# BioinformaticsArchive/HSA

Measured on AMD Instinct MI355X. Metric: aligned reads/sec, 100bp synthetic vs hg19-sized 2BWT, at 1/2/4/8 MI355X, higher is better.
Workload: dtype u32

## Files before the change

### hsa_amd/csrc/hsa_index.hip

```cpp
#include <chrono>
#include <cstring>
#include <hip/hip_runtime.h>
#include <rocprim/rocprim.hpp>
#include <stdarg.h>
#include <stdio.h>
#include <stdlib.h>
#include <string.h>

#include "hsa_device.h"
#include "hsa_internal.h"
#include "hsa_trie.h"

static thread_local char g_err[1024] = "";
int g_waves_per_cu = 16;
int g_pool_entries = 0;
int g_batch_k = getenv("HSA_BATCH_K") ? atoi(getenv("HSA_BATCH_K")) : 32;
int g_batch_idle = getenv("HSA_BATCH_IDLE") ? atoi(getenv("HSA_BATCH_IDLE")) : 768;
int g_hit_cap = 64;

void hsa_set_error(const char *fmt, ...)
{
    va_list ap;
    va_start(ap, fmt);
    vsnprintf(g_err, sizeof g_err, fmt, ap);
    va_end(ap);
}

extern "C" const char *hsa_last_error(void) { return g_err; }
extern "C" void hsa_gpu_set_error_text(const char *msg) { hsa_set_error("%s", msg); }

extern "C" int hsa_device_count(void)
{
    int n = 0;
    if (hipGetDeviceCount(&n) != hipSuccess) return 0;
    return n;
}

extern "C" void hsa_free(void *p) { free(p); }

extern "C" int hsa_configure(int waves_per_cu, int pool_entries, int hit_cap)
{
    if (waves_per_cu > 0) g_waves_per_cu = waves_per_cu;
    if (pool_entries > 0) {
        if (pool_entries > 65535) { hsa_set_error("pool_entries > 65535"); return HSA_E_ARG; }
        g_pool_entries = pool_entries;
    } else if (pool_entries < 0) {
        g_pool_entries = 0;
    }
    if (hit_cap > 0) g_hit_cap = hit_cap;
    return 0;
}

static void hsa_log_alloc(const char *what, size_t bytes, std::chrono::steady_clock::time_point t0)
{
    const double ms = std::chrono::duration<double, std::milli>(std::chrono::steady_clock::now() - t0).count();
    if (ms > 5.0 && getenv("HSA_VERBOSE")) fprintf(stderr, "[hsa] %s: hipMalloc of %.2f GB took %.1f ms\n", what, bytes / 1e9, ms);
}

int hsa_realloc_device(void **out, void **old, size_t bytes)
{
    *out = nullptr;
    if (hipMalloc(out, bytes) != hipSuccess) {
        (void)hipGetLastError();
        *out = nullptr;
        (void)hipFree(*old);
        *old = nullptr;
        if (hipMalloc(out, bytes) != hipSuccess) {
            (void)hipGetLastError();
            *out = nullptr;
            hsa_set_error("hipMalloc(%zu) failed", bytes);
            return HSA_E_MEM;
        }
        return 0;
    }
    (void)hipFree(*old);
    *old = nullptr;
    return 0;
}

int hsa_grow(void **p, size_t *cap, size_t need)
{
    if (need <= *cap && *p) return 0;
    size_t n = need + need / 4 + 4096;
    const auto t0 = std::chrono::steady_clock::now();
    void *np = nullptr;
    *cap = 0;
    if (hsa_realloc_device(&np, p, n)) return HSA_E_MEM;
    *p = np;
    *cap = n;
    hsa_log_alloc("buffer", n, t0);
    return 0;
}

void hsa_scratch_free(SearchScratch &s)
{
    (void)hipFree(s.pool); (void)hipFree(s.nxt); (void)hipFree(s.hbuf);
    const size_t lb = s.link_bytes;
    s = SearchScratch();
    s.link_bytes = lb;
}

extern "C" int hsa_index_release_scratch(hsa_index_t *ix)
{
    if (!ix) { hsa_set_error("hsa_index_release_scratch: null handle"); return HSA_E_ARG; }
    (void)hipSetDevice(ix->device);
    HSA_HIP(hipStreamSynchronize(ix->stream));
    hsa_scratch_free(ix->main); hsa_scratch_free(ix->big); hsa_scratch_free(ix->huge);
    void **bufs[] = {&ix->d_pf, &ix->d_pf2, &ix->d_sp, &ix->d_any, &ix->d_any_aux, &ix->d_help, &ix->d_hp, &ix->d_rf,
                     &ix->d_ch, &ix->d_sm};
    size_t *caps[] = {&ix->d_pf_cap, &ix->d_pf2_cap, &ix->d_sp_cap, &ix->d_any_cap, &ix->d_any_aux_cap, &ix->d_help_cap,
                      &ix->d_hp_cap, &ix->d_rf_cap, &ix->d_ch_cap, &ix->d_sm_cap};
    for (int i = 0; i < 10; ++i) {
        if (*bufs[i]) (void)hipFree(*bufs[i]);
        *bufs[i] = nullptr;
        *caps[i] = 0;
    }
    return 0;
}

int hsa_scratch_reserve(SearchScratch &s, size_t lanes, size_t pcap, size_t hcap, size_t link_bytes)
{
    const size_t pe = lanes * pcap, he = lanes * hcap;
    auto fail = [&]() {
        hsa_set_error("scratch allocation failed (lanes %zu, pool %zu, hits %zu)", lanes, pcap, hcap);
        (void)hipGetLastError();
        hsa_scratch_free(s);
        return HSA_E_MEM;
    };
    if (!s.pool || pe > s.pool_entries || link_bytes != s.link_bytes) {
        const size_t npe = pe > s.pool_entries ? pe : s.pool_entries;
        const auto t0 = std::chrono::steady_clock::now();
        void *np = nullptr, *nn = nullptr;
        if (hsa_realloc_device(&np, (void **)&s.pool, npe * sizeof(uint4)) ||
            hsa_realloc_device(&nn, &s.nxt, npe * link_bytes)) {
            (void)hipFree(np);
            return fail();
        }
        s.pool = (uint4 *)np; s.nxt = nn;
        s.pool_entries = npe;
        s.link_bytes = link_bytes;
        hsa_log_alloc("search scratch pool", npe * (sizeof(uint4) + link_bytes), t0);
    }
    if (!s.hbuf || he > s.hit_entries) {
        const size_t nhe = he > s.hit_entries ? he : s.hit_entries;
        const auto t0 = std::chrono::steady_clock::now();
        void *nh = nullptr;
        if (hsa_realloc_device(&nh, (void **)&s.hbuf, nhe * 9 * sizeof(uint32_t))) return fail();
        s.hbuf = (uint32_t *)nh;
        s.hit_entries = nhe;
        hsa_log_alloc("search scratch hits", nhe * 9 * sizeof(uint32_t), t0);
    }
    return 0;
}

__global__ void k_msb_to_lsb(uint32_t *w, size_t n, uint32_t T)
{
    size_t i = (size_t)blockIdx.x * blockDim.x + threadIdx.x;
    if (i >= n) return;
    uint32_t x = w[i];
    x = (x >> 16) | (x << 16);
    x = ((x & 0xFF00FF00u) >> 8) | ((x & 0x00FF00FFu) << 8);
    x = ((x & 0xF0F0F0F0u) >> 4) | ((x & 0x0F0F0F0Fu) << 4);
    x = ((x & 0xCCCCCCCCu) >> 2) | ((x & 0x33333333u) << 2);
    if (i == n - 1 && (T & 15)) x &= (1u << (2 * (T & 15))) - 1u;
    w[i] = x;
}

// ... 711 lines not shown
```

### hsa_amd/csrc/hsa_search.hip

```cpp
#include "hsa_search_launch.h"
#include "hsa_splice_prefetch.h"

#include <memory>
#include <vector>

#ifdef HSA_DIAG
extern "C" int hsa_diag_read(unsigned long long *out, int n_blocks)
{
    HSA_HIP(hipMemcpyFromSymbol(out, HIP_SYMBOL(g_diag), sizeof(unsigned long long) * 4 * (size_t)n_blocks));
    return 0;
}
extern "C" int hsa_diag_counters(unsigned long long *out, int reset)
{
    HSA_HIP(hipMemcpyFromSymbol(out, HIP_SYMBOL(g_dctr), sizeof(unsigned long long) * 32));
    if (reset) {
        unsigned long long z[32] = {0};
        HSA_HIP(hipMemcpyToSymbol(HIP_SYMBOL(g_dctr), z, sizeof z));
    }
    return 0;
}
#endif

struct MgHost {
    const hsa_mg_job_t *mg;
// ... 112 lines not shown
}

static int export_widths(const HostIn &in, const HostStage &H)
{
    const MgHost *mh = in.mh;
    std::vector<int32_t> cw(2 * mh->width_pairs + 2);
    HSA_HIP(hipMemcpy(cw.data(), H.io.mg.d_cw, mh->width_pairs * 8, hipMemcpyDeviceToHost));
    for (int j = 0; j < in.n; ++j)
        memcpy(mh->widths_out + 2 * mh->mg[j].wb_off, cw.data() + 2 * mh->mg[j].wb_off, 8 * ((size_t)in.jobs[j].len + 1));
    return 0;
}

static void add_stats(hsa_stats_t *stats, const unsigned long long *ctr, float ms, bool main)
{
    if (!stats) return;
    stats->rank_queries += ctr[CTR_RANK]; stats->blocks_loaded += ctr[CTR_SECTORS]; stats->pops += ctr[CTR_POPS];
    stats->kernel_ms += ms;
    if (main) { stats->main_kernel_ms += ms; stats->main_launches += 1; }
}

static long search_any_host(hsa_index_t *ix, const hsa_regime_t *regimes, int n_regimes, const HostIn &in,
                            const HostOut &out)
{
    HSA_HIP(hipSetDevice(ix->device));
    hipStream_t st = ix->stream;
    const hsa_job_t *jobs = in.jobs;
    uint32_t max_len = 1, max_seed = 0;
    for (int j = 0; j < in.n; ++j) {
        if (jobs[j].len > max_len) max_len = jobs[j].len;
        const bool own = in.mh ? in.mh->mg[j].seed == HSA_SEED_OWN : (int)jobs[j].len > jobs[j].seed_len;
        if (own && (uint32_t)jobs[j].seed_len > max_seed) max_seed = (uint32_t)jobs[j].seed_len;
    }
    AnyBufs AB;
    int rc = any_prepare(ix, regimes, n_regimes, (size_t)in.n, st, AB);
    if (rc) return rc;
    HostStage H;
    if ((rc = stage_host(ix, in, nullptr, 0, st, H))) return rc;
    H.io.max_len = (int)max_len; H.io.max_seed = (int)max_seed;
    HSA_HIP(hipMemsetAsync(H.io.ctr, 0, CTR_SLOTS * sizeof(unsigned long long), st));
    HSA_HIP(hipEventRecord(ix->ev0, st));
    if ((rc = any_passes<uint32_t>(ix, AB, H.io, nullptr, st))) return rc;
    HSA_HIP(hipEventRecord(ix->ev1, st));
    unsigned long long ctr[CTR_SLOTS];
    if ((rc = copy_back(H.io, in.n, out, ctr, st))) return rc;
    if (ctr[CTR_ERRORS]) { hsa_set_error("%llu reads pushed a score past the regime's n_stacks", ctr[CTR_ERRORS]); return HSA_E_ARG; }
    if (ctr[CTR_UNFINISHED]) { hsa_set_error("%llu reads exceed the large-pass capacity", ctr[CTR_UNFINISHED]); return HSA_E_ARG; }
    float ms = 0;
    HSA_HIP(hipEventElapsedTime(&ms, ix->ev0, ix->ev1));
    const uint64_t total = ctr[CTR_HITS] < H.io.hit_cap ? ctr[CTR_HITS] : H.io.hit_cap;
    HostHits h = alloc_hits(total);
    if (!h) return HSA_E_MEM;
    if (total) HSA_HIP(hipMemcpy(h.get(), H.io.hits, total * 36, hipMemcpyDeviceToHost));
    if (in.mh && (rc = export_widths(in, H))) return rc;
    add_stats(out.stats, ctr, ms, true);
    *out.hits = h.release();
    return (long)total;
}

static long search_batch_impl(hsa_index_t *ix, const hsa_regime_t *regimes, int n_regimes, const HostIn &in,
                              const HostOut &out);

static long search_split(hsa_index_t *ix, const hsa_regime_t *regimes, int n_regimes, const HostIn &in, const HostOut &out,
                         bool fast_rg)
{
    const MgHost *mh = in.mh;
    hsa_stats_t *stats = out.stats;
    std::vector<int> part[2];
    for (int j = 0; j < in.n; ++j) part[fast_rg && in.jobs[j].len <= FAST_MAX_LEN ? 0 : 1].push_back(j);
    HostHits hs[2] = {HostHits(nullptr, free), HostHits(nullptr, free)};
    long tot[2] = {0, 0};
    if (stats) memset(stats, 0, sizeof *stats);
    for (int k = 0; k < 2; ++k) {
        const int m = (int)part[k].size();
        if (m == 0) continue;
        std::vector<hsa_job_t> pj(m);
        std::vector<hsa_mg_job_t> pm(mh ? m : 0);
        for (int q = 0; q < m; ++q) {
            pj[q] = in.jobs[part[k][q]];
            if (mh) pm[q] = mh->mg[part[k][q]];
        }
        const MgHost pmh = mh ? MgHost{pm.data(), mh->widths, mh->width_pairs, mh->widths_out} : MgHost{};
        std::vector<int32_t> na(m);
        std::vector<uint32_t> fl(m);
        std::vector<uint64_t> ho(m);
        hsa_stats_t ps{};
        uint32_t *ph = nullptr;
        const HostIn pin{pj.data(), m, in.codes, in.codes_len, mh ? &pmh : nullptr};
        const HostOut pout{na.data(), fl.data(), ho.data(), &ph, &ps};
        const long t = k == 0 ? search_batch_impl(ix, regimes, n_regimes, pin, pout)
                              : search_any_host(ix, regimes, n_regimes, pin, pout);
        hs[k].reset(ph);
        if (t < 0) return t;
        tot[k] = t;
        for (int q = 0; q < m; ++q) {
            const int j = part[k][q];
            out.n_aln[j] = na[q]; out.flags[j] = fl[q]; out.hit_off[j] = ho[q] + (k ? (uint64_t)tot[0] : 0);
        }
        if (stats) {
            stats->rank_queries += ps.rank_queries; stats->blocks_loaded += ps.blocks_loaded; stats->pops += ps.pops;
            stats->overflow_reruns += ps.overflow_reruns; stats->kernel_ms += ps.kernel_ms;
            stats->main_kernel_ms += ps.main_kernel_ms; stats->main_launches += ps.main_launches;
        }
    }
    HostHits h = alloc_hits((uint64_t)tot[0] + (uint64_t)tot[1]);
    if (!h) return HSA_E_MEM;
    if (tot[0]) memcpy(h.get(), hs[0].get(), (size_t)tot[0] * 36);
    if (tot[1]) memcpy(h.get() + (size_t)tot[0] * 9, hs[1].get(), (size_t)tot[1] * 36);
    *out.hits = h.release();
    return tot[0] + tot[1];
}

static long search_batch_impl(hsa_index_t *ix, const hsa_regime_t *regimes, int n_regimes, const HostIn &in,
                              const HostOut &out)
{
    const hsa_job_t *jobs = in.jobs;
    const int n_jobs = in.n;
    const size_t codes_len = in.codes_len;
    const MgHost *mh = in.mh;
    hsa_stats_t *stats = out.stats;
    *out.hits = nullptr;
    if (n_regimes < 1 || n_regimes > 2) { hsa_set_error("1 or 2 regimes"); return HSA_E_ARG; }
    if (int rc0 = hsa_need32(ix)) return rc0;
    int rc = check_regimes(regimes, n_regimes);
    if (rc) return rc;
    int max_len, max_seed;
    if ((rc = jobs_limits(jobs, n_jobs, max_len, max_seed))) return rc;
    if (mh && (rc = mg_limits(jobs, mh->mg, n_jobs, *mh, max_seed))) return rc;
    if (codes_len >= 0xFFFFFFFFull) { hsa_set_error("read codes of one call must be < 4 GiB"); return HSA_E_ARG; }
    HSA_HIP(hipSetDevice(ix->device));
    for (int j = 0; j < n_jobs; ++j)
        if (jobs[j].off > codes_len || jobs[j].len > codes_len - jobs[j].off) {
            hsa_set_error("job %d: codes [%llu, +%u) past codes_len %zu", j, (unsigned long long)jobs[j].off,
                          jobs[j].len, codes_len);
            return HSA_E_ARG;
        }
    const bool fast_rg = fast_regimes(regimes, n_regimes);
    bool all_fit = fast_rg;
    for (int j = 0; j < n_jobs && all_fit; ++j) all_fit = jobs[j].len <= FAST_MAX_LEN;
    if (!all_fit) return search_split(ix, regimes, n_regimes, in, out, fast_rg);
    hipStream_t st = ix->stream;
    if (stats) memset(stats, 0, sizeof *stats);
    if (n_jobs == 0) { *out.hits = (uint32_t *)calloc(9, 4); return 0; }
    static const bool verbose = getenv("HSA_VERBOSE") != nullptr;
    const auto now = []() { struct timespec t; clock_gettime(CLOCK_MONOTONIC, &t); return t.tv_sec + 1e-9 * t.tv_nsec; };
    const double tv0 = verbose ? now() : 0.0;

    HostStage H;
    if ((rc = stage_host(ix, in, regimes, n_regimes, st, H))) return rc;
    H.io.max_len = max_len; H.io.max_seed = max_seed;
    LaunchPlan P;
    RegimePlan R = regime_plan(regimes, n_regimes);
    R.nb = H.nb;
    R.nib_ok = R.nib_ok && !mh;
    for (int j = 0; j < n_jobs && R.nib_ok; ++j) R.nib_ok = jobs[j].max_diff <= 6;
    if ((rc = plan_launch(ix, n_jobs, max_len, max_seed, R, PASS_MAIN, P))) return rc;
    HSA_HIP(hipEventRecord(ix->ev0, st));
    if ((rc = launch_pass(ix, P, ix->main, H.io, PassLink{}, st))) return rc;
    HSA_HIP(hipEventRecord(ix->ev1, st));
    unsigned long long ctr[CTR_SLOTS];
    if ((rc = copy_back(H.io, n_jobs, out, ctr, st))) return rc;
    if (ctr[CTR_ERRORS]) { hsa_set_error("%llu reads exceed the regime's max_diff bound", ctr[CTR_ERRORS]); return HSA_E_ARG; }
    float ms = 0;
    HSA_HIP(hipEventElapsedTime(&ms, ix->ev0, ix->ev1));
    uint64_t total = ctr[CTR_HITS] < H.io.hit_cap ? ctr[CTR_HITS] : H.io.hit_cap;
    const double tv1 = verbose ? now() : 0.0;
    HostHits h = alloc_hits(total);
    if (!h) return HSA_E_MEM;
    if (total) HSA_HIP(hipMemcpy(h.get(), H.io.hits, total * 36, hipMemcpyDeviceToHost));
    if (verbose)
        fprintf(stderr, "[hsa] search of %d reads: copies in + kernels + result arrays out %.1f ms (kernels %.1f ms), "
                        "hits out %.1f ms\n", n_jobs, 1e3 * (tv1 - tv0), ms, 1e3 * (now() - tv1));
    add_stats(stats, ctr, ms, true);

    std::vector<int32_t> list, n2;
    std::vector<uint32_t> f2;
    std::vector<uint64_t> o2;
    for (int round = 0; round < 4; ++round) {
        list.clear();
        for (int j = 0; j < n_jobs; ++j) if (out.flags[j] & HSA_F_OVERFLOW) list.push_back(j);
        const int n_over = (int)list.size();
        if (n_over == 0) break;
        n2.resize(n_jobs); f2.resize(n_jobs); o2.resize(n_jobs);
        if (stats) stats->overflow_reruns += n_over;
        LaunchPlan B;
        const int mode = round == 0 ? PASS_BIG : PASS_HUGE;
        if ((rc = plan_launch(ix, n_over, max_len, max_seed, R, mode, B))) return rc;
        const uint64_t cap2 = (uint64_t)n_over * 256 * (round + 1) + 65536;
        const size_t o2_fl = al((size_t)n_jobs * 4), o2_ho = o2_fl * 2, o2_hits = o2_ho + al((size_t)n_jobs * 8);
        DevBuf d2;
        HSA_HIP(hipMalloc(&d2.p, o2_hits + cap2 * 36));
        HSA_HIP(hipMemcpyAsync(H.d_list, list.data(), sizeof(int32_t) * n_over, hipMemcpyHostToDevice, st));
        char *c2 = (char *)d2.p;
        PassIO io2 = H.io;
        io2.list = H.d_list; io2.n = n_over;
        io2.n_aln = (int32_t *)c2; io2.flags = (uint32_t *)(c2 + o2_fl); io2.hit_off = (uint64_t *)(c2 + o2_ho);
        io2.hits = (uint32_t *)(c2 + o2_hits); io2.hit_cap = cap2;
        HSA_HIP(hipEventRecord(ix->ev0, st));
        if ((rc = launch_pass(ix, B, mode == PASS_BIG ? ix->big : ix->huge, io2, PassLink{}, st))) return rc;
        HSA_HIP(hipEventRecord(ix->ev1, st));
        if ((rc = copy_back(io2, n_jobs, HostOut{n2.data(), f2.data(), o2.data(), nullptr, nullptr}, ctr, st))) return rc;
        HSA_HIP(hipEventElapsedTime(&ms, ix->ev0, ix->ev1));
        const uint64_t t2 = ctr[CTR_HITS] < cap2 ? ctr[CTR_HITS] : cap2;
        uint32_t *grown = (uint32_t *)realloc(h.get(), (total + t2 + 1) * 36);
        if (!grown) { hsa_set_error("host allocation of %llu hits failed", (unsigned long long)(total + t2)); return HSA_E_MEM; }
        (void)h.release(); h.reset(grown);
        if (t2) HSA_HIP(hipMemcpy(h.get() + total * 9, io2.hits, t2 * 36, hipMemcpyDeviceToHost));
        for (const int j : list) { out.n_aln[j] = n2[j]; out.flags[j] = f2[j]; out.hit_off[j] = o2[j] + total; }
        total += t2;
        add_stats(stats, ctr, ms, false);
    }
    for (int j = 0; j < n_jobs; ++j)
        if (out.flags[j] & HSA_F_OVERFLOW) { hsa_set_error("read %d exceeds the large-pass capacity", j); return HSA_E_ARG; }
    if (mh && (rc = export_widths(in, H))) return rc;
    *out.hits = h.release();
    return (long)total;
}

extern "C" long hsa_search_batch(hsa_index_t *ix, const hsa_regime_t *regimes, int n_regimes, const hsa_job_t *jobs,
                                 int n_jobs, const uint8_t *codes, size_t codes_len, int32_t *n_aln, uint32_t *flags,
                                 uint64_t *hit_off, uint32_t **hits_out, hsa_stats_t *stats)
{
    return search_batch_impl(ix, regimes, n_regimes, HostIn{jobs, n_jobs, codes, codes_len, nullptr},
                             HostOut{n_aln, flags, hit_off, hits_out, stats});
}

extern "C" long hsa_match_gap_batch(hsa_index_t *ix, const hsa_regime_t *regimes, int n_regimes, const hsa_job_t *jobs,
                                    const hsa_mg_job_t *mg, int n_jobs, const uint8_t *codes, size_t codes_len,
                                    const int32_t *widths, size_t width_pairs, int32_t *widths_out, int32_t *n_aln,
                                    uint64_t *hit_off, uint32_t **hits_out, hsa_stats_t *stats)
{
    *hits_out = nullptr;
    if (n_jobs > 0 && (!mg || !widths || !widths_out)) { hsa_set_error("hsa_match_gap_batch: null argument"); return HSA_E_ARG; }
    std::vector<uint32_t> flags((size_t)(n_jobs > 0 ? n_jobs : 0) + 1);
    const MgHost mh{mg, widths, width_pairs, widths_out};
    return search_batch_impl(ix, regimes, n_regimes, HostIn{jobs, n_jobs, codes, codes_len, &mh},
                             HostOut{n_aln, flags.data(), hit_off, hits_out, stats});
}

extern "C" int hsa_search_device(hsa_index_t *ix, const hsa_regime_t *regimes, int n_regimes,
                                 const hsa_device_batch_t *b, void *stream)
{
    if (int rc = hsa_need32(ix)) return rc;
    return search_device_impl<uint32_t>(ix, regimes, n_regimes, b, stream);
}

extern "C" int hsa_pass_times(hsa_index_t *ix, int n, float *widths_ms, float *search_ms)
{
    if (n < 1 || n > hsa_index::PASS_RING || (uint64_t)n > ix->pev_n) {
        hsa_set_error("hsa_pass_times: %d passes requested, %llu recorded (ring %d)", n,
                      (unsigned long long)ix->pev_n, hsa_index::PASS_RING);
        return HSA_E_ARG;
    }
    for (int i = 0; i < n; ++i) {
        hipEvent_t *pe = ix->pev[(ix->pev_n - (uint64_t)n + (uint64_t)i) % hsa_index::PASS_RING];
        HSA_HIP(hipEventSynchronize(pe[2]));
        HSA_HIP(hipEventElapsedTime(widths_ms + i, pe[0], pe[1]));
        HSA_HIP(hipEventElapsedTime(search_ms + i, pe[1], pe[2]));
    }
    return 0;
}

extern "C" int hsa_last_pass_ms(hsa_index_t *ix, float *widths_ms, float *search_ms)
{
    if (ix->pev_n) return hsa_pass_times(ix, 1, widths_ms, search_ms);
    HSA_HIP(hipEventSynchronize(ix->ev1));
    HSA_HIP(hipEventElapsedTime(widths_ms, ix->ev0, ix->evm));
    HSA_HIP(hipEventElapsedTime(search_ms, ix->evm, ix->ev1));
    return 0;
}
```

### hsa_amd/csrc/hsa_search_kernels.h

```cpp
#pragma once
#include <hip/hip_runtime.h>
#include <stdio.h>
#include <stdlib.h>
#include <string.h>

#include <type_traits>

#include "hsa_device.h"
#include "hsa_internal.h"
#include "hsa_trie.h"

#define NIL16 0xFFFFu
#define BLOCK 256
#define MAXB 128
#define MAXS 512

enum : uint32_t { PH_IDLE = 0, PH_POP, PH_EXACT, PH_EXPAND, PH_EXIT, PH_END, PH_WAIT };

struct SearchArgs {
    RankDir fwd, rev;
    uint32_t T;
    uint32_t C[5];
    RankDir64 fwd64, rev64;
    uint64_t T64;
    uint64_t C64[5];
    const hsa_regime_t *regimes;
    const uint8_t *bmap;
    uint32_t ntab;
    const hsa_job_t *jobs;
    const int32_t *job_list;
    int n_jobs;
    const uint8_t *codes;
    int32_t *n_aln;
    uint32_t *flags;
    uint64_t *hit_off;
    uint32_t *hits;
    uint64_t hit_cap;
    unsigned long long *ctr;
    const uint8_t *wb, *ws;
    uint32_t *wg;
    uint32_t rb, rs, rg;
    uint4 *pool;
    void *nxt;
    uint32_t *hbuf;
    uint32_t pcap, hcap, nb;
    uint32_t off_heads, off_wb, off_ws;
    uint32_t nib_wb, nib_ws;
    uint32_t mm_buckets;
    int32_t *ovf_list;
    const unsigned long long *n_dev;
    uint32_t qctr;
    uint32_t ovf_ctr;
    const hsa_mg_job_t *mg;
    int32_t *cw;
    int32_t *wbid;
    uint32_t *wq;
    uint32_t batch_k;
    uint32_t batch_idle;
    uint32_t split;
    int32_t *sp_n;
    uint64_t *sp_off;
    uint32_t *sp_q, *sp_p;
    const void *ktw;
    uint32_t ktd;
    uint8_t *wkey;
    const int32_t *perm;
    uint32_t okey;
    int32_t *fwd_list;
    unsigned long long *fwd_n;
    uint32_t fwd_only;
    int32_t *rmap;
    uint32_t fr_budget, fr_demand, fr_cap;
    uint32_t *fr_ent;
    uint32_t *fr_tag;
    uint32_t *fr_rq;
    uint32_t *fr_st;
    unsigned long long *fr_q, *fr_p;
    unsigned long long *fr_c;
    const void *stw;
    uint32_t sdc;
};
#define FR_HIT 0x80000000u
#define FR_DONE 0x40000000u
#define FR_EW 8u
#define FR_CH 16u
#define FR_WALK 1024u
#ifndef HSA_HELPERS
#define HSA_HELPERS 1
#endif

typedef const __attribute__((address_space(4))) SearchArgs *ColdArgs;
__device__ __forceinline__ ColdArgs cold_args()
{
    ColdArgs p = (ColdArgs)(__builtin_amdgcn_kernarg_segment_ptr());
    asm volatile("" : "+s"(p));
    return p;
}

__device__ __forceinline__ uint32_t meta_pack(uint32_t i, uint32_t st, uint32_t isd, uint32_t mm, uint32_t go,
                                              uint32_t ge)
{
    return i | st << 10 | isd << 12 | mm << 13 | go << 20 | ge << 24;
}
#define M_I(m) ((int)((m) & 1023u))
#define M_ST(m) ((int)(((m) >> 10) & 3u))
#define M_ISD(m) ((int)(((m) >> 12) & 1u))
#define M_MM(m) ((int)(((m) >> 13) & 127u))
#define M_GO(m) ((int)(((m) >> 20) & 15u))
#define M_GE(m) ((int)((m) >> 24))

#define C_PH(c) ((c) & 7u)
#define C_STRAND(c) (((c) >> 3) & 1u)
#define C_SEED(c) (((c) >> 4) & 1u)
#define C_REG(c) (((c) >> 5) & 1u)
#define C_VT(c) (((c) >> 6) & 1u)
#define C_ALIAS(c) (((c) >> 7) & 1u)
#define C_OVF(c) (((c) >> 8) & 3u)
#define C_LEN(c) ((int)(((c) >> 10) & 1023u))
#define C_SLEN(c) ((int)(((c) >> 20) & 1023u))
#define SET_PH(c, p) ((c) = ((c) & ~7u) | (p))

template <typename V>
__device__ __forceinline__ V pick4(const V v[4], uint32_t c)
{
    return hsa_sel4<V>(c, v[0], v[1], v[2], v[3]);
}

template <typename IT> struct Ix;
template <> struct Ix<uint32_t> {
    __device__ static const RankDir &fwd(const SearchArgs &a) { return a.fwd; }
    __device__ static const RankDir &rev(const SearchArgs &a) { return a.rev; }
    __device__ static uint32_t T(const SearchArgs &a) { return a.T; }
    __device__ static const uint32_t *C(const SearchArgs &a) { return a.C; }
};
template <> struct Ix<uint64_t> {
    __device__ static const RankDir64 &fwd(const SearchArgs &a) { return a.fwd64; }
    __device__ static const RankDir64 &rev(const SearchArgs &a) { return a.rev64; }
    __device__ static uint64_t T(const SearchArgs &a) { return a.T64; }
    __device__ static const uint64_t *C(const SearchArgs &a) { return a.C64; }
};

template <typename IT> struct Ent {
    IT x, y, z;
    uint32_t w;
};
#ifndef HSA_WAVES_SIMD
#define HSA_WAVES_SIMD 4
#endif
#ifndef HSA_POOL_CHUNK
#define HSA_POOL_CHUNK 1
#endif
template <typename IT>
__device__ __forceinline__ size_t pool_base(size_t wv, uint32_t pcap, int lane)
{
#if HSA_POOL_CHUNK
    return (sizeof(IT) == 4 ? 1u : 2u) * wv * (size_t)((pcap + 31u) & ~31u) * 64 + (size_t)lane * 4;
#else
    return (sizeof(IT) == 4 ? 1u : 2u) * wv * pcap * 64 + (size_t)lane;
#endif
}
template <typename IT>
__device__ __forceinline__ size_t ent_at(size_t base, uint32_t slot)
{
#if HSA_POOL_CHUNK
    constexpr uint32_t EQ = sizeof(IT) == 4 ? 4u : 2u, U = sizeof(IT) == 4 ? 1u : 2u;
    return base + (size_t)(slot / EQ) * 256 + (slot % EQ) * U;
#else
    return base + (size_t)slot * (sizeof(IT) == 4 ? 64 : 128);
#endif
}
template <typename IT>
__device__ __forceinline__ Ent<IT> ent_load(const uint4 *pool, size_t base, uint32_t slot)
{
    const size_t i = ent_at<IT>(base, slot);
    if constexpr (sizeof(IT) == 4) {
        const uint4 v = pool[i];
        return Ent<IT>{v.x, v.y, v.z, v.w};
    } else {
        const uint4 u = pool[i], v = pool[i + (HSA_POOL_CHUNK ? 1 : 64)];
        return Ent<IT>{(uint64_t)u.x | (uint64_t)u.y << 32, (uint64_t)u.z | (uint64_t)u.w << 32,
                       (uint64_t)v.x | (uint64_t)v.y << 32, v.z};
    }
}
template <typename IT>
__device__ __forceinline__ void ent_store(uint4 *pool, size_t base, uint32_t slot, const Ent<IT> &e)
{
    const size_t i = ent_at<IT>(base, slot);
    if constexpr (sizeof(IT) == 4) {
        pool[i] = make_uint4(e.x, e.y, e.z, e.w);
    } else {
        pool[i] = make_uint4((uint32_t)e.x, (uint32_t)(e.x >> 32), (uint32_t)e.y, (uint32_t)(e.y >> 32));
        pool[i + (HSA_POOL_CHUNK ? 1 : 64)] = make_uint4((uint32_t)e.z, (uint32_t)(e.z >> 32), e.w, 0u);
    }
}
template <typename IT> struct HitW { static constexpr uint32_t STAGE = sizeof(IT) == 4 ? 9u : 10u;
                                     static constexpr uint32_t OUT = sizeof(IT) == 4 ? 9u : 14u; };

template <int MW> struct BMask;
template <> struct BMask<0> {
    uint32_t m0 = 0;
    __device__ __forceinline__ void clear() { m0 = 0; }
    __device__ __forceinline__ bool any() const { return m0 != 0; }
    __device__ __forceinline__ int lowest() const { return m0 ? __ffs(m0) - 1 : (1 << 30); }
    __device__ __forceinline__ bool test(int b) const { return (m0 >> b) & 1u; }
    __device__ __forceinline__ void set(int b) { m0 |= 1u << b; }
    __device__ __forceinline__ void reset(int b) { m0 &= ~(1u << b); }
};
template <> struct BMask<1> {
    uint64_t m0 = 0;
    __device__ __forceinline__ void clear() { m0 = 0; }
    __device__ __forceinline__ bool any() const { return m0 != 0; }
    __device__ __forceinline__ int lowest() const { return m0 ? __ffsll((unsigned long long)m0) - 1 : (1 << 30); }
    __device__ __forceinline__ bool test(int b) const { return (m0 >> b) & 1ull; }
    __device__ __forceinline__ void set(int b) { m0 |= 1ull << b; }
    __device__ __forceinline__ void reset(int b) { m0 &= ~(1ull << b); }
};
template <> struct BMask<2> {
    uint64_t m0 = 0, m1 = 0;
    __device__ __forceinline__ void clear() { m0 = m1 = 0; }
    __device__ __forceinline__ bool any() const { return (m0 | m1) != 0; }
    __device__ __forceinline__ int lowest() const
    {
        if (m0) return __ffsll((unsigned long long)m0) - 1;
        if (m1) return 64 + __ffsll((unsigned long long)m1) - 1;
        return 1 << 30;
    }
    __device__ __forceinline__ bool test(int b) const { return b < 64 ? ((m0 >> b) & 1ull) : ((m1 >> (b - 64)) & 1ull); }
    __device__ __forceinline__ void set(int b) { if (b < 64) m0 |= 1ull << b; else m1 |= 1ull << (b - 64); }
    __device__ __forceinline__ void reset(int b) { if (b < 64) m0 &= ~(1ull << b); else m1 &= ~(1ull << (b - 64)); }
};

template <typename WT> struct WFmt {
    static constexpr bool NIB = false;
    static constexpr uint32_t BIDB = sizeof(WT) == 1 ? 4u : 8u;
    static constexpr uint32_t BIDM = (1u << BIDB) - 1u;
    static constexpr uint32_t EQ = 1u << BIDB;
    static constexpr uint32_t CSH = BIDB + 1u;
    static constexpr uint32_t EB = 8u * sizeof(WT);
    static constexpr uint32_t EPW = 4u / sizeof(WT);
    __device__ static uint32_t code_bits(uint32_t c) { return (c & 3u) << CSH | (c > 3 ? 4u : 0u) << CSH; }
    __device__ static uint32_t code(uint32_t v) { return (v >> CSH) & 7u; }
};

struct WNib { uint8_t v; };
template <> struct WFmt<WNib> {
    static constexpr bool NIB = true;
    static constexpr uint32_t BIDB = 3u, BIDM = 7u, EQ = 8u, EB = 4u, EPW = 8u;
};

__device__ __forceinline__ uint32_t nib4(uint32_t x)
{
    uint32_t b = x & 0x0F0F0F0Fu;
    const uint32_t ge7 = ((b + 0x09090909u) >> 4) & 0x01010101u;
    b = (b & ~(ge7 * 0x0Fu)) | ge7 * 7u;
    uint32_t n = b | ((x >> 4) & 0x01010101u) << 3;
    n = (n | n >> 4) & 0x00FF00FFu;
    return (n | n >> 8) & 0xFFFFu;
}

#ifdef HSA_DIAG
static __device__ unsigned long long g_diag[8192 * 4];
static __device__ unsigned long long g_dctr[32];
#define DC(i) (++dc[i])
#else
#define DC(i) ((void)0)
#endif

template <typename IT> struct WChain {
    IT k, l;
    uint32_t bid;
    IT prevw;
    uint32_t acc;
    uint32_t tl, tix;
    uint32_t lr;
};

template <typename WT, typename IT>
__device__ __forceinline__ void width_step(const SearchArgs &a, WChain<IT> &ch, uint32_t t, uint32_t n, uint32_t c,
                                           uint32_t cbits, uint32_t *__restrict__ brow, IT *__restrict__ wrow,
                                           uint32_t &st_q, uint32_t &st_b, uint32_t &st_t)
{
    using F = WFmt<WT>;
    IT w;
    if (t < n) {
        if (c < 4) {
            if (ch.tl < a.ktd) {
                ch.tix = ch.tix * 4u + c;
                ++ch.tl;
                trie_w_load<IT>(a.ktw, trie_base(ch.tl) + ch.tix, ch.k, ch.l);
                ++st_t;
            } else {
                IT ok, ol;
                st_b += occ1_pair(Ix<IT>::rev(a), ch.k, ch.l + 1u, c, ok, ol);
                const IT cc = pick4(Ix<IT>::C(a), c);
                ch.k = cc + ok + 1u;
                ch.l = cc + ol;
            }
            st_q += 2;
        }
        if (ch.k > ch.l || c > 3) { ch.k = 0; ch.l = Ix<IT>::T(a); ++ch.bid; ch.tl = 0; ch.tix = 0; ch.lr = t; }
        w = ch.l - ch.k + 1u;
    } else {
        w = 0; ++ch.bid;
    }
    if (t > 0) {
        if (ch.prevw == w) ch.acc |= F::EQ << (((t - 1) % F::EPW) * F::EB);
        if ((t - 1) % F::EPW == F::EPW - 1) { brow[((t - 1) / F::EPW) * 64] = ch.acc; ch.acc = 0; }
    }
    ch.acc |= ((ch.bid < F::BIDM ? ch.bid : F::BIDM) | cbits) << ((t % F::EPW) * F::EB);
    if (wrow) wrow[t * 64] = w;
    ch.prevw = w;
    if (t == n) brow[(t / F::EPW) * 64] = ch.acc;
}

struct WRow { uint32_t q, b, t, bid, tail; };

__device__ __forceinline__ uint8_t cost_key(const SearchArgs &a, const WRow &w)
{
    const uint32_t b = w.bid < 15u ? w.bid : 15u;
    if (!a.okey) return (uint8_t)(w.bid < 255u ? w.bid : 255u);
    return (uint8_t)(b << 4 | (w.tail < 16u ? 2u : w.tail < 48u ? 1u : 0u));
}

template <typename WT, typename IT>
__device__ __forceinline__ WRow width_row(const SearchArgs &a, uint32_t R, uint32_t strand, const hsa_job_t &J)
{
    using F = WFmt<WT>;
    const uint32_t len = J.len;
    const uint64_t off = J.off;
    const bool has_seed = (int)len > J.seed_len;
    const uint32_t slen = has_seed ? (uint32_t)J.seed_len : 0u;
    const size_t rb = R >> 6, rl = R & 63u;
    uint32_t *const brow = reinterpret_cast<uint32_t *>(const_cast<uint8_t *>(a.wb)) + rb * (a.rb / 4) * 64 + rl;
    uint32_t *const srow = reinterpret_cast<uint32_t *>(const_cast<uint8_t *>(a.ws)) + rb * (a.rs / 4) * 64 + rl;
    IT *const wrow = reinterpret_cast<IT *>(a.wg) + rb * a.rg * 64 + rl;
    WChain<IT> f{0, Ix<IT>::T(a), 0, 0, 0, 0, 0}, sd{0, Ix<IT>::T(a), 0, 0, 0, 0, 0};
    uint32_t st_q = 0, st_b = 0, st_t = 0;
    const uint32_t s0 = len - slen;
#ifndef HSA_CODECACHE
#define HSA_CODECACHE 1
#endif
    uint32_t cq[2] = {0xFFFFFFFFu, 0xFFFFFFFFu}, cword[2] = {0u, 0u};
    auto base = [&](uint32_t sp, int ch) -> uint32_t {
        const uint64_t ix = off + (strand ? len - 1u - sp : sp);
        uint32_t c;
        if constexpr (HSA_CODECACHE) {
            const uint32_t wq = (uint32_t)(ix >> 2);
            if (wq != cq[ch]) {
                cword[ch] = *reinterpret_cast<const uint32_t *>(a.codes + (ix & ~(uint64_t)3));
                cq[ch] = wq;
            }
            c = (cword[ch] >> (((uint32_t)ix & 3u) * 8u)) & 0xFFu;
        } else {
            c = a.codes[ix];
        }
        return strand && c < 4 ? 3u - c : c;
    };
    for (uint32_t t = 0; t <= len; ++t) {
        const uint32_t cf = t < len ? base(t, 0) : 4u;
        width_step<WT, IT>(a, f, t, len, cf, t < len ? F::code_bits(cf) : 0u, brow, wrow, st_q, st_b, st_t);
        if (has_seed && t <= slen) {
            const uint32_t cs = t < slen ? base(s0 + t, 1) : 4u;
            width_step<WT, IT>(a, sd, t, slen, cs, 0u, srow, nullptr, st_q, st_b, st_t);
        }
    }
    return WRow{st_q, st_b, st_t, f.bid, len - f.lr};
}

__device__ __forceinline__ void wave_add(unsigned long long *c, unsigned long long v)
{
    for (int d = 32; d >= 1; d >>= 1) v += __shfl_xor(v, d);
    if ((threadIdx.x & 63) == 0 && v) atomicAdd(c, v);
}

#define HSA_NOFWD 0xFFFFFFFFu
#define HSA_F_NEEDFWD 0x100u

template <typename WT, typename IT = uint32_t>
__global__ void __launch_bounds__(BLOCK) k_widths(SearchArgs a)
{
    const uint32_t R = blockIdx.x * BLOCK + threadIdx.x;
    const uint32_t n_jobs = a.n_dev ? (uint32_t)*a.n_dev : (uint32_t)a.n_jobs;
    const uint32_t q = R >> 1, strand = R & 1u;
    WRow w{0, 0, 0, 0};
    if (R < 2u * n_jobs) {
        const hsa_job_t J = a.jobs[a.job_list ? a.job_list[q] : (int)q];
        w = width_row<WT, IT>(a, R, strand, J);
        if (!strand) a.wq[q] = w.q;
        if (a.wkey) a.wkey[R] = cost_key(a, w);
    }
    wave_add(&a.ctr[CTR_RANK], strand ? w.q : 0u);
    wave_add(&a.ctr[CTR_WIDTH_Q], strand ? w.q : 0u);
    wave_add(&a.ctr[CTR_FWD_Q_ALL], strand ? 0u : w.q);
    wave_add(&a.ctr[CTR_SECTORS], w.b);
    wave_add(&a.ctr[CTR_TRIE], w.t);
}

template <typename WT, typename IT = uint32_t>
__global__ void __launch_bounds__(BLOCK) k_widths_reads(SearchArgs a, uint32_t mode, int32_t *list2,
                                                        unsigned long long *n2)
{
    const uint32_t p = blockIdx.x * BLOCK + threadIdx.x;
    const uint32_t n_jobs = mode == 3 ? (uint32_t)*n2 : a.n_dev ? (uint32_t)*a.n_dev : (uint32_t)a.n_jobs;
    WRow w{0, 0, 0, 0};
    bool more = false;
    if (p < n_jobs) {
        const uint32_t q = mode == 3 ? (uint32_t)list2[p] : p;
        const hsa_job_t J = a.jobs[a.job_list ? a.job_list[q] : (int)q];
        const uint32_t R = mode == 1 ? q : mode == 3 ? (uint32_t)(((uint32_t)a.n_jobs + 63u) & ~63u) + p : 2u * q;
        w = width_row<WT, IT>(a, R, mode == 1 ? 1u : 0u, J);
        if (mode == 3) a.rmap[q] = (int32_t)R;
        const uint8_t key = cost_key(a, w);
        if (mode == 1) {
            more = (int)w.bid - 1 > J.max_diff;
            a.wq[q] = HSA_NOFWD;
            if (a.wkey) { a.wkey[2 * q + 1] = key; a.wkey[2 * q] = 255u; }
        } else if (mode == 3) {
            a.wq[q] = w.q;
            if (a.wkey) a.wkey[2 * q] = key;
        }
    }
    if (mode == 1) {
        const uint64_t m = __ballot(more);
        const int lane = (int)(threadIdx.x & 63);
        unsigned long long b = 0;
        if (m && lane == __ffsll((unsigned long long)m) - 1) b = atomicAdd(n2, (unsigned long long)__popcll(m));
        b = __shfl(b, __ffsll((unsigned long long)(m ? m : 1ull)) - 1);
        if (more) list2[b + __popcll(m & ((1ull << lane) - 1ull))] = (int32_t)p;
    }
    const uint32_t rq = mode == 1 ? w.q : 0u, fq = mode == 2 ? w.q : 0u, sq = mode == 3 ? w.q : 0u;
    wave_add(&a.ctr[CTR_RANK], rq + fq);
    wave_add(&a.ctr[CTR_WIDTH_Q], rq + fq);
    wave_add(&a.ctr[CTR_FWD_Q_ALL], fq + sq);
    wave_add(&a.ctr[CTR_FWD_Q_REF], fq);
    wave_add(&a.ctr[CTR_SECTORS], w.b);
    wave_add(&a.ctr[CTR_TRIE], w.t);
}

template <typename WT>
__global__ void __launch_bounds__(BLOCK) k_widths_import(SearchArgs a)
{
    using F = WFmt<WT>;
    const uint32_t q = blockIdx.x * BLOCK + threadIdx.x;
    const uint32_t n_jobs = a.n_dev ? (uint32_t)*a.n_dev : (uint32_t)a.n_jobs;
    if (q >= n_jobs) return;
    const int job = a.job_list ? a.job_list[q] : (int)q;
    const hsa_job_t J = a.jobs[job];
    const hsa_mg_job_t M = a.mg[job];
    const uint32_t R = q * 2u + (uint32_t)(M.strand & 1);
    const size_t rb = R >> 6, rl = R & 63u;
    uint32_t *const brow = reinterpret_cast<uint32_t *>(const_cast<uint8_t *>(a.wb)) + rb * (a.rb / 4) * 64 + rl;
    uint32_t *const srow = reinterpret_cast<uint32_t *>(const_cast<uint8_t *>(a.ws)) + rb * (a.rs / 4) * 64 + rl;
    uint32_t *const wrow = a.wg + rb * a.rg * 64 + rl;
    int32_t *const drow = a.wbid + rb * a.rg * 64 + rl;
    const bool prefix = M.seed == HSA_SEED_ALIAS && M.ws_off == HSA_MG_PREFIX;
    auto emit = [&](uint32_t *row, const int32_t *w, uint32_t n, bool read_row) {
        uint32_t acc = 0;
        uint32_t wt = (uint32_t)w[0];
        for (uint32_t t = 0; t <= n; ++t) {
            const uint32_t bid = prefix && t == n ? (n ? (uint32_t)w[2 * t - 1] + 1u : 1u) : (uint32_t)w[2 * t + 1];
            const uint32_t wn = t + 1 < n || (t + 1 == n && !prefix) ? (uint32_t)w[2 * t + 2] : 0u;
            uint32_t e = bid < F::BIDM ? bid : F::BIDM;
            if (t < n && wt == wn) e |= F::EQ;
            if (read_row && t < n) e |= F::code_bits(a.codes[J.off + t]);
            acc |= e << ((t % F::EPW) * F::EB);
            if (t % F::EPW == F::EPW - 1 || t == n) { row[(t / F::EPW) * 64] = acc; acc = 0; }
            if (read_row) { wrow[t * 64] = wt; drow[t * 64] = (int32_t)bid; }
            wt = wn;
        }
    };
    emit(brow, a.cw + 2 * M.wb_off, J.len, true);
    if (M.seed == HSA_SEED_OWN) emit(srow, a.cw + 2 * M.ws_off, (uint32_t)J.seed_len, false);
}

static __global__ void __launch_bounds__(BLOCK) k_widths_export(SearchArgs a)
{
    const uint32_t q = blockIdx.x * BLOCK + threadIdx.x;
    const uint32_t n_jobs = a.n_dev ? (uint32_t)*a.n_dev : (uint32_t)a.n_jobs;
    if (q >= n_jobs) return;
    const int job = a.job_list ? a.job_list[q] : (int)q;
    if (a.flags[job] & HSA_F_OVERFLOW) return;
    const hsa_job_t J = a.jobs[job];
    const hsa_mg_job_t M = a.mg[job];
    if (M.seed == HSA_SEED_ALIAS && M.ws_off == HSA_MG_PREFIX) return;
    const uint32_t R = q * 2u + (uint32_t)(M.strand & 1);
    const size_t base = (R >> 6) * (size_t)a.rg * 64 + (R & 63u);
    int32_t *const o = a.cw + 2 * M.wb_off;
    for (uint32_t t = 0; t <= J.len; ++t) {
        o[2 * t] = (int32_t)a.wg[base + t * 64];
        o[2 * t + 1] = a.wbid[base + t * 64];
    }
}


__device__ __forceinline__ uint32_t order_bin(const SearchArgs &a, uint32_t q)
{
    const uint32_t k0 = a.wkey[2 * q], k1 = a.wkey[2 * q + 1];
    const uint32_t k = k0 < k1 ? k0 : k1;
    if (a.okey) {
        const uint32_t v = (k >> 4) * 3u + (k & 15u);
        return 15u - (v < 15u ? v : 15u);
    }
    return 15u - (k < 15u ? k : 15u);
}

static __global__ void __launch_bounds__(BLOCK) k_order_hist(SearchArgs a, uint32_t *hist)
{
    __shared__ uint32_t h[16];
    if (threadIdx.x < 16) h[threadIdx.x] = 0;
    __syncthreads();
    const uint32_t q = blockIdx.x * BLOCK + threadIdx.x;
    if (q < (uint32_t)a.n_jobs) atomicAdd(&h[order_bin(a, q)], 1u);
    __syncthreads();
    if (threadIdx.x < 16 && h[threadIdx.x]) atomicAdd(&hist[threadIdx.x], h[threadIdx.x]);
}

static __global__ void k_order_scan(uint32_t *hist)
{
    uint32_t s = 0;
    for (int b = 0; b < 16; ++b) { hist[16 + b] = s; s += hist[b]; }
}

static __global__ void __launch_bounds__(BLOCK) k_order_scatter(SearchArgs a, uint32_t *hist, int32_t *perm)
{
    __shared__ uint32_t h[16], base[16];
    if (threadIdx.x < 16) h[threadIdx.x] = 0;
    __syncthreads();
    const uint32_t q = blockIdx.x * BLOCK + threadIdx.x;
    uint32_t b = 0, r = 0;
    if (q < (uint32_t)a.n_jobs) { b = order_bin(a, q); r = atomicAdd(&h[b], 1u); }
    __syncthreads();
    if (threadIdx.x < 16 && h[threadIdx.x]) base[threadIdx.x] = atomicAdd(&hist[16 + threadIdx.x], h[threadIdx.x]);
    __syncthreads();
    if (q < (uint32_t)a.n_jobs) perm[base[b] + r] = (int32_t)q;
}

static __global__ void __launch_bounds__(BLOCK) k_split_finalize(SearchArgs a)
{
    const uint32_t q = blockIdx.x * BLOCK + threadIdx.x;
    const uint32_t n_jobs = a.n_dev ? (uint32_t)*a.n_dev : (uint32_t)a.n_jobs;
    unsigned long long q_add = 0, p_add = 0, w_add = 0;
    if (q < n_jobs) {
        const int job = a.job_list ? a.job_list[q] : (int)q;
        const int32_t nr = a.sp_n[2 * q], nf = a.sp_n[2 * q + 1];
        int32_t na = 0;
        uint32_t fl = 0;
        uint64_t off = 0;
        if (nr < 0 || (nr == 0 && nf < 0)) {
            fl = HSA_F_OVERFLOW;
            if (a.ovf_list) a.ovf_list[atomicAdd(&a.ctr[a.ovf_ctr], 1ull)] = job;
            else atomicAdd(&a.ctr[CTR_UNFINISHED], 1ull);
        } else if (nr > 0) {
            na = nr; off = a.sp_off[2 * q];
            q_add = a.sp_q[2 * q]; p_add = a.sp_p[2 * q];
        } else {
            w_add = a.wq[q];
            q_add = (unsigned long long)a.sp_q[2 * q] + a.sp_q[2 * q + 1] + w_add;
            p_add = (unsigned long long)a.sp_p[2 * q] + a.sp_p[2 * q + 1];
            if (nf > 0) { na = nf; off = a.sp_off[2 * q + 1]; }
            else fl = HSA_F_FALLBACK;
        }
        a.n_aln[job] = na;
        a.flags[job] = fl;
        a.hit_off[job] = off;
    }
    for (int d = 32; d >= 1; d >>= 1) {
        q_add += __shfl_xor(q_add, d);
        p_add += __shfl_xor(p_add, d);
        w_add += __shfl_xor(w_add, d);
    }
    if ((threadIdx.x & 63) == 0) {
        if (q_add) atomicAdd(&a.ctr[CTR_RANK], q_add);
        if (p_add) atomicAdd(&a.ctr[CTR_POPS], p_add);
        if (w_add) { atomicAdd(&a.ctr[CTR_WIDTH_Q], w_add); atomicAdd(&a.ctr[CTR_FWD_Q_REF], w_add); }
    }
}

template <int MW, bool GAPS, typename WT, int NT, bool HUGE = false, typename IT = uint32_t>
__global__ void __launch_bounds__(NT, HSA_WAVES_SIMD) k_search(SearchArgs a)
{
    using F = WFmt<WT>;
    using E = Ent<IT>;
    using CT = typename std::conditional<sizeof(IT) == 8, int64_t, int>::type;
    constexpr uint32_t HW = HitW<IT>::STAGE, OW = HitW<IT>::OUT;
    const IT TT = Ix<IT>::T(a);
    const IT *const CC = Ix<IT>::C(a);
    using LT = typename std::conditional<HUGE, uint32_t, uint16_t>::type;
    constexpr bool FRH = !HUGE && HSA_HELPERS && GAPS && sizeof(IT) == 4 && !WFmt<WT>::NIB;
    constexpr uint32_t NIL = HUGE ? 0xFFFFFFFFu : (uint32_t)NIL16;
    constexpr bool IMP = !GAPS && !HUGE && sizeof(IT) == 4 && !WFmt<WT>::NIB;
#ifdef HSA_DIAG
    if (threadIdx.x == 0 && blockIdx.x < 8192) {
        g_diag[blockIdx.x * 4 + 0] = __builtin_amdgcn_s_memtime();
        g_diag[blockIdx.x * 4 + 1] = __builtin_amdgcn_s_memrealtime();
    }
#endif
    extern __shared__ __align__(16) uint8_t s_lds[];
    const uint32_t tid = threadIdx.x;
    const uint32_t gid = blockIdx.x * NT + tid;
    const int lane = (int)(tid & 63);
    for (uint32_t t = tid; t < 2 * a.ntab; t += NT) s_lds[t] = a.bmap[(t / a.ntab) * MAXS + t % a.ntab];
    static_assert(2 * sizeof(hsa_regime_t) <= 128, "regime LDS slot");
    hsa_regime_t *const s_reg = reinterpret_cast<hsa_regime_t *>(s_lds + 2 * a.ntab);
    if (tid < 2 * sizeof(hsa_regime_t) / 4)
        reinterpret_cast<uint32_t *>(s_reg)[tid] = reinterpret_cast<const uint32_t *>(a.regimes)[tid];
    __syncthreads();
    LT *const s_heads = reinterpret_cast<LT *>(s_lds + a.off_heads);
    using WTL = typename std::conditional<F::NIB, uint8_t, WT>::type;
    WTL *const s_wb = reinterpret_cast<WTL *>(s_lds + a.off_wb);
    WTL *const s_ws = reinterpret_cast<WTL *>(s_lds + a.off_ws);
    uint32_t *const s_nb = reinterpret_cast<uint32_t *>(s_lds + a.off_wb);
    uint32_t *const s_ns = reinterpret_cast<uint32_t *>(s_lds + a.off_ws);
    const size_t wv = gid >> 6;
#if HSA_POOL_CHUNK
    const size_t link0 = wv * (size_t)((a.pcap + 31u) & ~31u) * 64 + (size_t)lane * 32;
#define NXT(s) reinterpret_cast<LT *>(a.nxt)[link0 + (size_t)((s) >> 5) * 2048 + ((s) & 31u)]
#else
    const size_t link0 = wv * a.pcap * 64 + (size_t)lane;
#define NXT(s) reinterpret_cast<LT *>(a.nxt)[link0 + (size_t)(s) * 64]
#endif
    const size_t pbase = pool_base<IT>(wv, a.pcap, lane);
#define HB(i) r->hbuf[(wv * r->hcap * HW + (uint32_t)(i)) * 64 + lane]
#define HEAD(b) s_heads[(uint32_t)(b) * NT + tid]
#define WB(p) s_wb[(((uint32_t)(p) / F::EPW) * NT + tid) * F::EPW + (uint32_t)(p) % F::EPW]
#define WS(p) s_ws[(((uint32_t)(p) / F::EPW) * NT + tid) * F::EPW + (uint32_t)(p) % F::EPW]
#define RG(f) (s_reg[C_REG(ctl)].f)

    uint32_t ctl = PH_IDLE;
    uint32_t qpos = 0;
    uint32_t pen = 0;
    uint32_t rmode = 0;
    uint32_t pos = 0;
    IT ik = 0, il = 0;
    IT aux = 0;
    int opt_max_diff = 0, max_diff = 0, best_score = 0, n_aln = 0, n_entries = 0;
    CT best_cnt = 0;
    uint32_t pool_top = 0;
    uint32_t free_head = NIL;
    uint32_t idle_acc = 0;
    BMask<MW> mask;
    E e{0, 0, 0, 0};
    uint32_t st_p = 0, st_wq = 0, st_q = 0, st_b = 0;
    uint32_t sq0 = 0, sp0 = 0;
    uint32_t frs = 0, fr_p0 = 0, fr_q0 = 0;
    uint32_t fr_tick = 0;
    uint32_t st_hs = 0, st_hq = 0;
    const uint32_t n_jobs = a.n_dev ? (uint32_t)*a.n_dev : (uint32_t)a.n_jobs;
#ifdef HSA_DIAG
    uint32_t dc[21] = {0};
    uint64_t tsec[4] = {0, 0, 0, 0};
    uint64_t tt = 0;
    uint64_t rd_t0 = 0;
    uint32_t rd_steps = 0, rd_p0 = 0;
#define TMARK(k) do { const uint64_t t_ = __builtin_amdgcn_s_memtime(); tsec[k] += t_ - tt; tt = t_; } while (0)
#endif

#define S_MM ((int)(pen & 1023u))
#define S_GO ((int)((pen >> 10) & 1023u))
#define S_GE ((int)(pen >> 20))
#define R_MODE ((int)(rmode & 255u))
#define R_MAXGO ((int)((rmode >> 8) & 255u))
#define R_MAXGE ((int)(rmode >> 16))
#define SCORE(mm, go, ge) ((mm) * S_MM + (go) * S_GO + (ge) * S_GE)

    auto wbg = [&](int p) -> uint32_t {
        if constexpr (F::NIB) return (s_nb[((uint32_t)p >> 3) * NT + tid] >> (((uint32_t)p & 7u) * 4u)) & 15u;
        else return WB(p);
    };
    auto wsg = [&](int p) -> uint32_t {
        if constexpr (F::NIB) return (s_ns[((uint32_t)p >> 3) * NT + tid] >> (((uint32_t)p & 7u) * 4u)) & 15u;
        else return WS(p);
    };
    auto wbs = [&](int p, uint32_t v) {
        if constexpr (F::NIB) {
            uint32_t &w = s_nb[((uint32_t)p >> 3) * NT + tid];
            const uint32_t sh = ((uint32_t)p & 7u) * 4u;
            w = (w & ~(15u << sh)) | v << sh;
        } else {
            WB(p) = (WTL)v;
        }
    };
    const uint8_t *rowp = nullptr;
    uint32_t cur_c = 0;
#ifndef HSA_ROWCACHE
#define HSA_ROWCACHE 1
#endif
    uint32_t rw_q = 0xFFFFFFFFu, rw_w = 0;
    auto getc = [&](int p) -> uint32_t {
        if constexpr (F::NIB && !HSA_ROWCACHE) {
            return WFmt<uint8_t>::code(rowp[((uint32_t)p >> 2) * 256u + ((uint32_t)p & 3u)]);
        } else if constexpr (F::NIB) {
            const uint32_t q = (uint32_t)p >> 2;
            if (q != rw_q) {
                rw_w = *reinterpret_cast<const uint32_t *>(rowp + q * 256u);
                rw_q = q;
            }
            return WFmt<uint8_t>::code((rw_w >> (((uint32_t)p & 3u) * 8u)) & 0xFFu);
        } else {
            return F::code(WB(p));
        }
    };
    auto bucket_of = [&](uint32_t m) -> int {
        if (!GAPS && a.mm_buckets) return M_MM(m);
        const int sc = SCORE(M_MM(m), M_GO(m), M_GE(m));
        return (uint32_t)sc < a.ntab ? (int)s_lds[C_REG(ctl) * a.ntab + sc] : 0xFF;
    };
    auto flush = [&](const E &v, int b) {
        if ((uint32_t)b >= a.nb) { ctl |= 1u << 8; return; }
        uint32_t slot;
        if (HUGE && free_head != NIL) {
            slot = free_head;
            free_head = NXT(slot);
        } else {
            if (pool_top >= a.pcap) { ctl |= 1u << 8; return; }
            slot = pool_top++;
        }
        DC(8);
        ent_store<IT>(a.pool, pbase, slot, v);
        const uint32_t old = mask.test(b) ? (uint32_t)HEAD(b) : NIL;
        NXT(slot) = (LT)old;
        HEAD(b) = (LT)slot;
        mask.set(b);
    };
    auto start_search = [&]() {
        best_score = SCORE(opt_max_diff + 1, R_MAXGO + 1, R_MAXGE + 1);
        max_diff = opt_max_diff;
        best_cnt = 0; n_aln = 0;
        mask.clear(); pool_top = 0; free_head = NIL;
        e = E{0, TT, 0, meta_pack((uint32_t)C_LEN(ctl), ST_M, 0, 0, 0, 0)};
        ctl |= 1u << 6;
        n_entries = 1;
        frs = 0; fr_p0 = st_p;
        SET_PH(ctl, PH_POP);
    };
    auto fr_key = [&]() -> uint32_t { return qpos * 2u + (1u - C_STRAND(ctl)); };
    auto row_base = [&](uint32_t cap_words) -> size_t {
        const int32_t *const rm = cold_args()->rmap;
        const uint32_t r = rm ? (C_STRAND(ctl) ? qpos : (uint32_t)rm[qpos]) : qpos * 2u + C_STRAND(ctl);
        return (size_t)(r >> 6) * cap_words * 64 + (r & 63u);
    };
    auto start_strand = [&]() {
        const ColdArgs r = cold_args();
        const uint32_t *src = reinterpret_cast<const uint32_t *>(r->wb) + row_base(r->rb / 4);
        const uint32_t nwb = r->rb / 4;
        if constexpr (F::NIB) {
            rowp = reinterpret_cast<const uint8_t *>(src);
            rw_q = 0xFFFFFFFFu;
            auto pack = [&](const uint32_t *row, uint32_t nw, uint32_t *dst, uint32_t cap) {
                const uint32_t nn = (nw + 1u) / 2u < cap ? (nw + 1u) / 2u : cap;
                for (uint32_t j = 0; j < nn; j += 4) {
                    uint32_t w[8];
#pragma unroll
                    for (uint32_t u = 0; u < 8; ++u) w[u] = 2u * j + u < nw ? row[(2u * j + u) * 64u] : 0u;
#pragma unroll
                    for (uint32_t u = 0; u < 4; ++u)
                        if (j + u < nn) dst[(j + u) * NT + tid] = nib4(w[2u * u]) | nib4(w[2u * u + 1u]) << 16;
                }
            };
            pack(src, nwb, s_nb, r->nib_wb);
            if (C_SEED(ctl) && !C_ALIAS(ctl))
                pack(reinterpret_cast<const uint32_t *>(r->ws) + row_base(r->rs / 4), r->rs / 4, s_ns, r->nib_ws);
        } else {
        uint32_t *const db = reinterpret_cast<uint32_t *>(s_wb) + (tid & ~63u);
        for (uint32_t q = 0; q < nwb; ++q)
            __builtin_amdgcn_global_load_lds(src + q * 64, db + q * NT, 4, 0, 0);
        if (C_SEED(ctl) && !C_ALIAS(ctl)) {
            const uint32_t *ss = reinterpret_cast<const uint32_t *>(r->ws) + row_base(r->rs / 4);
            uint32_t *const ds = reinterpret_cast<uint32_t *>(s_ws) + (tid & ~63u);
            const uint32_t nws = r->rs / 4;
            for (uint32_t q = 0; q < nws; ++q)
                __builtin_amdgcn_global_load_lds(ss + q * 64, ds + q * NT, 4, 0, 0);
        }
        }
        __builtin_amdgcn_s_waitcnt(0);
        DC(15);
        start_search();
    };
    auto finish_job = [&](uint32_t fl, int na, uint64_t ho) {
        const ColdArgs r = cold_args();
#ifdef HSA_DIAG
        atomicMax(&g_dctr[21], (unsigned long long)rd_steps);
        atomicMax(&g_dctr[22], (unsigned long long)(__builtin_amdgcn_s_memrealtime() - rd_t0));
        atomicMax(&g_dctr[23], (unsigned long long)(st_p - rd_p0));
        atomicMax(&g_dctr[na > 0 ? 24 : 25], (unsigned long long)rd_steps);
#endif
        if (r->split) {
            const uint32_t pi = qpos * 2u + (1u - C_STRAND(ctl));
            r->sp_n[pi] = (fl & HSA_F_OVERFLOW) ? -1 : na;
            r->sp_off[pi] = ho;
            r->sp_q[pi] = st_q - sq0;
            r->sp_p[pi] = st_p - sp0;
            st_q = sq0; st_p = sp0;
            if constexpr (FRH) {
                if (a.fr_budget) {
                    if (frs & 1u) atomicOr(&r->fr_st[pi], FR_DONE);
                    atomicAdd(&r->fr_c[2], 1ull);
                    frs = 0;
                }
            }
            SET_PH(ctl, PH_IDLE);
            return;
        }
        const int job = r->job_list ? r->job_list[qpos] : (int)qpos;
        if (fl & HSA_F_NEEDFWD) {
            r->fwd_list[atomicAdd(r->fwd_n, 1ull)] = job;
            SET_PH(ctl, PH_IDLE);
            return;
        }
        if (fl & HSA_F_OVERFLOW) {
            if (r->ovf_list) r->ovf_list[atomicAdd(&r->ctr[r->ovf_ctr], 1ull)] = job;
            else atomicAdd(&r->ctr[CTR_UNFINISHED], 1ull);
        }
        r->n_aln[job] = na;
        r->flags[job] = fl;
        r->hit_off[job] = ho;
        SET_PH(ctl, PH_IDLE);
    };
    auto help_done = [&]() {
        const ColdArgs r = cold_args();
        const uint32_t key = fr_key();
        const unsigned long long dq = st_q - fr_q0, dp = st_p - fr_p0;
        st_q = fr_q0; st_p = fr_p0;
        const unsigned long long o1 = atomicAdd(&r->fr_q[key], dq), o2 = atomicAdd(&r->fr_p[key], dp);
        asm volatile("s_waitcnt vmcnt(0)" :: "v"(o1), "v"(o2) : "memory");
        atomicSub(&r->fr_st[key], 1u);
        ++st_hs; st_hq += (uint32_t)dq;
        frs = 0;
        SET_PH(ctl, PH_IDLE);
    };
    auto end_strand = [&]() {
        if constexpr (FRH) {
            if (frs & 2u) { help_done(); return; }
        }
        if (n_aln > 0) {
            const ColdArgs r = cold_args();
            const unsigned long long o = atomicAdd(&r->ctr[CTR_HITS], (unsigned long long)n_aln);
            if (o + (uint64_t)n_aln > r->hit_cap) { finish_job(HSA_F_OVERFLOW, 0, 0); return; }
            uint32_t *dst = r->hits + o * OW;
            const uint32_t s30 = C_STRAND(ctl) << 30;
            for (int h = 0; h < n_aln; ++h) {
                const uint32_t end = h == 0 && !r->mg ? (uint32_t)(C_LEN(ctl) - 1) : 0u;
                if constexpr (sizeof(IT) == 4) {
                    const uint32_t v0 = HB(h * 9 + 0), v1 = HB(h * 9 + 1), v2 = HB(h * 9 + 2), v3 = HB(h * 9 + 3),
                                   v4 = HB(h * 9 + 4), v8 = HB(h * 9 + 8);
                    dst[h * 9 + 0] = v0;
                    dst[h * 9 + 1] = v1;
                    dst[h * 9 + 2] = v2;
                    dst[h * 9 + 3] = v3;
                    dst[h * 9 + 4] = v4;
                    dst[h * 9 + 5] = s30;
                    dst[h * 9 + 6] = 0;
                    dst[h * 9 + 7] = end;
                    dst[h * 9 + 8] = v8;
                } else {
                    uint32_t v[10];
#pragma unroll
                    for (int j = 0; j < 10; ++j) v[j] = HB(h * 10 + j);
                    dst[h * 14 + 0] = v[0];
                    dst[h * 14 + 1] = s30;
#pragma unroll
                    for (int j = 1; j < 9; ++j) dst[h * 14 + 1 + j] = v[j];
                    dst[h * 14 + 10] = 0;
                    dst[h * 14 + 11] = end;
                    dst[h * 14 + 12] = v[9];
                    dst[h * 14 + 13] = 0;
                }
            }
            finish_job(0, n_aln, o);
        } else if (cold_args()->mg || cold_args()->split) {
            finish_job(0, 0, 0);
        } else if (C_STRAND(ctl)) {
            const uint32_t wq = cold_args()->wq[qpos];
            if (wq == HSA_NOFWD) {
                finish_job(HSA_F_NEEDFWD, 0, 0);
            } else {
                ctl &= ~(1u << 3);
                st_wq += wq;
                start_strand();
            }
        } else {
            finish_job(HSA_F_FALLBACK, 0, 0);
        }
    };
    auto on_hit = [&](IT k, IT l, IT rk, IT rl) -> bool {
        const ColdArgs r = cold_args();
        if constexpr (FRH) {
            if (frs & 3u) {
                atomicOr(&r->fr_st[fr_key()], FR_HIT);
                if (frs & 2u) return false;
            }
        }
        const uint32_t m = e.w;
        const int score = SCORE(M_MM(m), M_GO(m), M_GE(m));
        if (n_aln == 0) {
            best_score = score;
            const int best_diff = M_MM(m) + M_GO(m) + ((R_MODE & MODE_GAPE) ? M_GE(m) : 0);
            if (!(R_MODE & MODE_NONSTOP)) max_diff = (best_diff + 1 > opt_max_diff) ? opt_max_diff : best_diff + 1;
        }
        if (score == best_score) {
            if constexpr (sizeof(IT) == 4) best_cnt = (int)((uint32_t)best_cnt + (l - k + 1u));
            else best_cnt += (CT)(l - k + 1u);
        } else if (best_cnt > RG(max_top2)) {
            return false;
        }
        bool add = true;
        if (M_GO(m)) {
            for (int j = 0; j < n_aln; ++j) {
                if constexpr (sizeof(IT) == 4) {
                    if (HB(j * 9 + 1) == k && HB(j * 9 + 2) == l) { add = false; break; }
                } else {
                    const uint64_t hk = (uint64_t)HB(j * 10 + 1) | (uint64_t)HB(j * 10 + 2) << 32;
                    const uint64_t hl = (uint64_t)HB(j * 10 + 3) | (uint64_t)HB(j * 10 + 4) << 32;
                    if (hk == k && hl == l) { add = false; break; }
                }
            }
        }
        if (add) {
            if ((uint32_t)n_aln >= r->hcap) { ctl |= 1u << 8; return false; }
            const IT x = l - k + 1u;
            const int ldp = M_ISD(m) ? M_I(m) : 0;
            if (ldp > 0) {
#ifdef HSA_DIAG
// ... 308 lines not shown
                    const uint64_t em = __ballot(elig);
                    if (elig && lane == __ffsll((unsigned long long)em) - 1) {
                        const unsigned long long wt = __hip_atomic_load(&r->fr_c[3], __ATOMIC_RELAXED, __HIP_MEMORY_SCOPE_AGENT);
                        const unsigned long long rs = __hip_atomic_load(&r->fr_c[0], __ATOMIC_RELAXED, __HIP_MEMORY_SCOPE_AGENT);
                        const unsigned long long tk = __hip_atomic_load(&r->fr_c[1], __ATOMIC_RELAXED, __HIP_MEMORY_SCOPE_AGENT);
                        if (wt > rs - tk + a.fr_demand) {
                            if (!fr_offer()) frs |= 4u;
                            else if (frs & 2u) stop = true;
                            else { frs |= 1u; fr_p0 = st_p; fr_q0 = st_q; }
                        }
                    }
                    if (stop) { SET_PH(ctl, PH_END); continue; }
                }
            }
            if (C_VT(ctl)) {
                DC(3);
                ctl &= ~(1u << 6);
            } else {
                DC(4);
                const int b = mask.lowest();
                const uint32_t slot = HEAD(b);
                e = ent_load<IT>(a.pool, pbase, slot);
                const uint32_t nx = NXT(slot);
                if (nx == NIL) mask.reset(b);
                else HEAD(b) = (LT)nx;
                if (HUGE) { NXT(slot) = (LT)free_head; free_head = slot; }
            }
            --n_entries;
            ++st_p;
            const uint32_t m = e.w;
            if (!(R_MODE & MODE_NONSTOP) && SCORE(M_MM(m), M_GO(m), M_GE(m)) > best_score + S_MM) {
                SET_PH(ctl, PH_END);
                continue;
            }
            const int em = m_of(m);
            if (em < 0) { DC(18); continue; }
            const int ei = M_I(m);
            if (ei > 0 && em < (int)(wbg(ei - 1) & F::BIDM)) { DC(18); continue; }
            if (ei == 0) {
                DC(20);
                if (!on_hit(e.x, e.y, e.z, e.z + (e.y - e.x)) && !C_OVF(ctl)) SET_PH(ctl, PH_END);
                continue;
            }
            if (em == 0 && (M_ST(m) == ST_M || (R_MODE & MODE_GAPE) || M_GE(m) == R_MAXGE)) {
                ik = e.x; il = e.y; aux = e.z + (e.y - e.x); pos = (uint32_t)(ei - 1);
                SET_PH(ctl, PH_EXACT);
                continue;
            }
            req = 1; rp1 = e.x; rp2 = e.y + 1u;
            if constexpr (IMP) {
                const uint32_t len = (uint32_t)C_LEN(ctl), dp = len - (uint32_t)ei;
                if (len > a.sdc && dp < a.sdc) req = dp + 1u == a.sdc ? 2 : 4;
            }
            if constexpr (F::NIB) cur_c = getc(ei - 1);
            SET_PH(ctl, PH_EXPAND);
        } while (0);

#ifdef HSA_DIAG
        TMARK(1);
#endif
        IT oa[4], ob[4], srk[4];
#ifdef HSA_DIAG
        {
            const uint64_t rq = __ballot(req == 1);
            if (lane == 0) dc[6] += (uint32_t)__popcll(rq);
            const uint32_t ph0 = C_PH(ctl);
            if (req == 1) DC(ph0 == PH_EXACT ? 1 : 2);
            if (req == 1 && rp2 == rp1 + 1u) DC(ph0 == PH_EXACT ? 16 : 17);
        }
#endif
        uint32_t two = 0;
#ifdef HSA_DIAG
        rd_steps += req == 1 ? 1u : 0u;
#endif
        if constexpr (IMP) {
            if (req == 2) {
                trie_s_load4(a.stw, rp1, oa, ob, srk);
            } else if (req == 3) {
                trie_s_load1(a.stw, rp1, oa[0], ob[0], srk[0]);
            }
        }
        if (req == 1) {
            two = occ_pair(Ix<IT>::fwd(a), rp1, rp2, oa, ob) - 1u;
            st_q += 2u; st_b += 1u + two;
        }

#ifdef HSA_DIAG
        asm volatile("s_waitcnt vmcnt(0)" ::: "memory");
        TMARK(2);
#endif
        const uint32_t ph = C_PH(ctl);
        if (IMP && req == 3) {
            ik = oa[0]; il = ob[0]; aux = srk[0] + (il - ik);
            if (M_I(e.w) != C_LEN(ctl)) e.x = e.y = e.z = 1u;
            --pos;
        } else if (F::NIB && req == 1 && ph == PH_EXACT && cur_c > 3) {
            st_q -= 2u; st_b -= 1u + two;
            SET_PH(ctl, PH_POP);
        } else if (req && ph == PH_EXACT) {
            const uint32_t c = F::NIB ? cur_c : getc((int)pos);
            IT oc = 0;
#pragma unroll
            for (uint32_t d = 1; d < 4; ++d) oc += d > c ? ob[d] - oa[d] : (IT)0;
            const IT cc = pick4(CC, c);
            ik = cc + pick4(oa, c) + 1u;
            il = cc + pick4(ob, c);
            aux -= oc;
            if (ik > il) {
                SET_PH(ctl, PH_POP);
            } else if (pos-- == 0) {
                const IT rk = aux - (il - ik), erl = e.z + (e.y - e.x);
                const IT hk = e.x ? ik : (IT)0, hl = e.y ? il : (IT)0, hrk = e.z ? rk : (IT)0, hrl = erl ? aux : (IT)0;
                SET_PH(ctl, PH_POP);
                if (!on_hit(hk, hl, hrk, hrl) && !C_OVF(ctl)) SET_PH(ctl, PH_END);
            }
        } else if (req && ph == PH_EXPAND) {
            const uint32_t m = e.w;
            const IT ek = e.x, el = e.y, erk = e.z, erl = erk + (el - ek);
            const int i = M_I(m) - 1;
            const int est = M_ST(m), emm = M_MM(m), ego = M_GO(m), ege = M_GE(m);
            const int em = m_of(m);
            const int len = C_LEN(ctl);
            uint32_t ne = 0;
            if (IMP && req != 1) {
                if (req == 4) {
#pragma unroll
                    for (int c = 0; c < 4; ++c) { oa[c] = ek * 4u + (IT)c; ob[c] = 0; srk[c] = 0; }
                }
                ne = 0xFu;
                st_q += 2u;
            } else {
                IT oc = 0;
#pragma unroll
                for (int c = 3; c >= 0; --c) {
                    const IT d = ob[c] - oa[c];
                    oa[c] = CC[c] + oa[c] + 1u;
                    ob[c] = CC[c] + ob[c];
                    srk[c] = (erl - oc) - (ob[c] - oa[c]);
                    oc += d;
                }
#pragma unroll
                for (int c = 0; c < 4; ++c) ne |= (oa[c] <= ob[c] ? 1u : 0u) << c;
            }
            int allow_diff = 1, allow_M = 1;
            if (i > 0) {
                const uint32_t w1 = wbg(i - 1), w0 = wbg(i);
                const int b1 = (int)(w1 & F::BIDM), b0 = (int)(w0 & F::BIDM);
                if (b1 > em - 1) allow_diff = 0;
                else if (b1 == em - 1 && b0 == em - 1 && (w1 & F::EQ)) allow_M = 0;
                const int ii = i - (len - C_SLEN(ctl));
                if (C_SEED(ctl) && ii > 0) {
                    int ems = RG(max_seed_diff) - (emm + ego);
                    if (R_MODE & MODE_GAPE) ems -= ege;
                    const uint32_t s1 = C_ALIAS(ctl) ? wbg(ii - 1) : wsg(ii - 1);
                    const uint32_t s0 = C_ALIAS(ctl) ? wbg(ii) : wsg(ii);
                    const int c1 = (int)(s1 & F::BIDM), c0 = (int)(s0 & F::BIDM);
                    if (c1 > ems - 1) allow_diff = 0;
                    else if (c1 == ems - 1 && c0 == ems - 1 && (s1 & F::EQ)) allow_M = 0;
                }
            }
            const uint32_t sc = F::NIB ? cur_c : getc(i);
            uint32_t cand = 0;
            if constexpr (GAPS) {
                const int ies = RG(indel_end_skip);
                const int tmp = (R_MODE & MODE_LOGGAP) ? hsa_log2((uint32_t)(ege + ego)) / 2 + 1 : ego + ege;
                const bool ok = (allow_diff != 0) & ((R_MAXGO > 0) | (ego > 0)) & (i >= ies + tmp) & (len - i >= ies + tmp);
                const IT occ = el - ek + 1u;
                const uint32_t c_m = ego < R_MAXGO ? (1u | ne << 1) : 0u;
                const uint32_t c_i = ege < R_MAXGE ? 1u : 0u;
                const bool d_ok = (ege < R_MAXGE) & ((ege + ego < max_diff) | (occ < (IT)RG(max_del_occ)));
                const uint32_t c_d = d_ok ? ne << 1 : 0u;
                const uint32_t c_g = est == ST_M ? c_m : est == ST_I ? c_i : c_d;
                cand = ok ? c_g : 0u;
            }
            {
                uint32_t c_mm = 0;
#pragma unroll
                for (int j = 1; j <= 4; ++j) {
                    const uint32_t c = (sc + (uint32_t)j) & 3u;
                    c_mm |= ((ne >> c) & 1u) << (4 + j);
                }
                const uint32_t c_eq = sc < 4 ? ((ne >> (sc & 3u)) & 1u) << 8 : 0u;
                cand |= (allow_diff & allow_M) ? c_mm : c_eq;
            }
            auto entry = [&](uint32_t b) -> E {
                const bool ins = GAPS && b == 0, del = GAPS && b >= 1 && b <= 4;
                const uint32_t c = del ? b - 1u : (sc + b - 4u) & 3u;
                const uint32_t is_mm = (b != 8u || sc > 3) ? 1u : 0u;
                IT k = pick4(oa, c), l = pick4(ob, c), rk = pick4(srk, c);
                uint32_t meta;
                if (GAPS && (ins || del)) {
                    if (ins) { k = ek; l = el; rk = erk; }
                    const uint32_t go = (uint32_t)ego + (est == ST_M), ge = (uint32_t)ege + (est != ST_M);
                    meta = meta_pack((uint32_t)(del ? i + 1 : i), ins ? ST_I : ST_D, 1u, (uint32_t)emm, go, ge);
                } else {
                    meta = meta_pack((uint32_t)i, ST_M, is_mm, (uint32_t)emm + is_mm, (uint32_t)ego, (uint32_t)ege);
                }
                return E{k, l, rk, meta};
            };
#ifdef HSA_DIAG
            auto doomed = [&](uint32_t mw) {
                const int em2 = m_of(mw), i2 = M_I(mw);
                return em2 < 0 || (i2 > 0 && em2 < (int)(wbg(i2 - 1) & F::BIDM));
            };
#endif
            if (cand) {
                const uint32_t last = 31u - (uint32_t)__clz(cand);
                n_entries += __popc(cand);
                uint32_t rest = cand & ~(1u << last);
                if constexpr (HUGE) {
                    for (; rest; rest &= rest - 1u) {
                        const E v = entry((uint32_t)__ffs(rest) - 1u);
#ifdef HSA_DIAG
                        if (doomed(v.w)) DC(19);
#endif
                        flush(v, bucket_of(v.w));
                    }
                } else if (rest) {
                    const uint32_t g_go = (uint32_t)ego + (est == ST_M), g_ge = (uint32_t)ege + (est != ST_M);
                    const uint32_t mI = meta_pack((uint32_t)i, ST_I, 1u, (uint32_t)emm, g_go, g_ge);
                    const uint32_t mD = meta_pack((uint32_t)(i + 1), ST_D, 1u, (uint32_t)emm, g_go, g_ge);
                    const uint32_t mM = meta_pack((uint32_t)i, ST_M, 1u, (uint32_t)emm + 1u, (uint32_t)ego, (uint32_t)ege);
                    const uint32_t mP = meta_pack((uint32_t)i, ST_M, 0u, (uint32_t)emm, (uint32_t)ego, (uint32_t)ege);
                    const int bG = GAPS ? bucket_of(mI) : -1, bM = bucket_of(mM), bP = bucket_of(mP);
                    auto head0 = [&](int b) -> uint32_t {
                        return b >= 0 && (uint32_t)b < a.nb && mask.test(b) ? (uint32_t)HEAD(b) : NIL;
                    };
                    const uint32_t hG0 = GAPS ? head0(bG) : NIL, hM0 = head0(bM), hP0 = head0(bP);
                    uint32_t hG = hG0, hM = hM0, hP = hP0;
                    for (; rest; rest &= rest - 1u) {
                        const uint32_t b = (uint32_t)__ffs(rest) - 1u;
                        const bool ins = GAPS && b == 0, gap = GAPS && b <= 4u;
                        const bool mt = b == 8u && sc < 4;
                        const uint32_t c = gap ? b - 1u : (sc + b - 4u) & 3u;
                        IT k = pick4(oa, c), l = pick4(ob, c), rk = pick4(srk, c);
                        if (ins) { k = ek; l = el; rk = erk; }
                        const uint32_t meta = ins ? mI : gap ? mD : mt ? mP : mM;
                        const int bk = gap ? bG : mt ? bP : bM;
#ifdef HSA_DIAG
                        if (doomed(meta)) DC(19);
#endif
                        if ((uint32_t)bk >= a.nb || pool_top >= a.pcap) { ctl |= 1u << 8; continue; }
                        const uint32_t slot = pool_top++;
                        DC(8);
                        ent_store<IT>(a.pool, pbase, slot, E{k, l, rk, meta});
                        NXT(slot) = (LT)(bk == bG ? hG : bk == bM ? hM : hP);
                        hG = bk == bG ? slot : hG;
                        hM = bk == bM ? slot : hM;
                        hP = bk == bP ? slot : hP;
                    }
                    if (GAPS && hG != hG0) { HEAD(bG) = (LT)hG; mask.set(bG); }
                    if (hM != hM0) { HEAD(bM) = (LT)hM; mask.set(bM); }
                    if (hP != hP0) { HEAD(bP) = (LT)hP; mask.set(bP); }
                }
                const E v = entry(last);
#ifdef HSA_DIAG
                if (doomed(v.w)) DC(19);
#endif
                const int bk = bucket_of(v.w);
                if (bk <= mask.lowest()) { e = v; ctl |= 1u << 6; }
                else flush(v, bk);
            }
            SET_PH(ctl, PH_POP);
        }
#ifdef HSA_DIAG
        TMARK(3);
#endif
    }

#ifdef HSA_DIAG
    __syncthreads();
    if (threadIdx.x == 0 && blockIdx.x < 8192) {
        g_diag[blockIdx.x * 4 + 2] = __builtin_amdgcn_s_memtime();
        g_diag[blockIdx.x * 4 + 3] = __builtin_amdgcn_s_memrealtime();
    }
    for (int i = 0; i < 18; ++i)
        if (i < 9 || i > 12) atomicAdd(&g_dctr[i], (unsigned long long)dc[i]);
    for (int i = 18; i < 21; ++i) atomicAdd(&g_dctr[i], (unsigned long long)dc[i]);
    if (lane == 0)
        for (int i = 0; i < 4; ++i) atomicAdd(&g_dctr[9 + i], (unsigned long long)tsec[i]);
#endif
    if constexpr (FRH) {
        if (a.fr_budget) {
            unsigned long long hs = st_hs, hq = st_hq;
            for (int d = 32; d >= 1; d >>= 1) { hs += __shfl_xor(hs, d); hq += __shfl_xor(hq, d); }
            if (lane == 0) { atomicAdd(&a.fr_c[6], hs); atomicAdd(&a.fr_c[8], hq); }
        }
    }
    atomicAdd(&a.ctr[CTR_RANK], (unsigned long long)st_q);
    atomicAdd(&a.ctr[CTR_SECTORS], (unsigned long long)st_b);
    atomicAdd(&a.ctr[CTR_POPS], (unsigned long long)st_p);
    if (st_wq) {
        atomicAdd(&a.ctr[CTR_RANK], (unsigned long long)st_wq);
        atomicAdd(&a.ctr[CTR_WIDTH_Q], (unsigned long long)st_wq);
        atomicAdd(&a.ctr[CTR_FWD_Q_REF], (unsigned long long)st_wq);
    }
#undef HEAD
#undef WB
#undef WS
#undef NXT
#undef HB
#undef RG
#undef S_MM
#undef S_GO
#undef S_GE
#undef R_MODE
#undef R_MAXGO
#undef R_MAXGE
#undef SCORE
}

// ... 11 lines not shown
```

### hsa_amd/csrc/hsa_search_launch.h

```cpp
#pragma once
#include "hsa_search_kernels.h"

static int check_regimes(const hsa_regime_t *rg, int n)
{
    for (int r = 0; r < n; ++r) {
        const hsa_regime_t &R = rg[r];
        if (R.s_mm < 0 || R.s_gapo < 0 || R.s_gape < 0) { hsa_set_error("negative penalty"); return HSA_E_ARG; }
        if (R.n_stacks <= 0 || R.n_stacks > ANY_MAX_STACKS) {
            hsa_set_error("n_stacks %d outside 1..%d", R.n_stacks, ANY_MAX_STACKS);
            return HSA_E_ARG;
        }
        if (R.max_gapo < 0 || R.max_gape < 0) { hsa_set_error("max_gapo/max_gape negative"); return HSA_E_ARG; }
        if (R.max_diff < -1) { hsa_set_error("max_diff out of range"); return HSA_E_ARG; }
    }
    return 0;
}

static int bucket_map(const hsa_regime_t &R, uint8_t map[MAXS])
{
    bool used[MAXS] = {false};
    const int md = R.max_diff < 0 ? 0 : R.max_diff;
    const int go_max = R.max_gapo < md ? R.max_gapo : md;
    for (int mm = 0; mm <= md + 1; ++mm)
        for (int go = 0; go <= go_max; ++go)
            for (int ge = 0; ge <= (go > 0 ? R.max_gape : 0); ++ge) {
                const int s = mm * R.s_mm + go * R.s_gapo + ge * R.s_gape;
                if (s >= 0 && s < MAXS && s < R.n_stacks) used[s] = true;
            }
    int k = 0;
    for (int s = 0; s < MAXS; ++s) map[s] = used[s] && k < 0xFF ? (uint8_t)k++ : (uint8_t)0xFF;
    return k;
}

static bool fast_regimes(const hsa_regime_t *rg, int n)
{
    if (getenv("HSA_FORCE_ANY")) return false;
    for (int r = 0; r < n; ++r) {
        const hsa_regime_t &R = rg[r];
        if (R.max_gapo > 14 || R.max_gape > 254 || R.max_diff > 125 || R.max_seed_diff > 254 || R.n_stacks > MAXS)
            return false;
        uint8_t map[MAXS];
        if (bucket_map(R, map) > MAXB) return false;
    }
    return true;
}

#define FAST_MAX_LEN 1023u

static bool mm_buckets(const hsa_regime_t *rg, int n, const uint8_t *bmap)
{
    for (int r = 0; r < n; ++r) {
        const hsa_regime_t &R = rg[r];
        if (R.max_gapo != 0 || R.s_mm <= 0) return false;
        const int md = R.max_diff < 0 ? 0 : R.max_diff;
        for (int mm = 0; mm <= md + 1; ++mm) {
            const int sc = mm * R.s_mm;
            if (sc >= MAXS || bmap[r * MAXS + sc] != mm) return false;
        }
    }
    return true;
}

struct RegimePlan {
    int nb;
    bool gaps, wide, nib_ok;
    int max_entries;
};

static RegimePlan regime_plan(const hsa_regime_t *rg, int n)
{
    RegimePlan C{.nb = 0, .gaps = false, .wide = false, .nib_ok = true, .max_entries = 0};
    for (int r = 0; r < n; ++r) {
        const int bound = rg[r].max_diff > rg[r].max_seed_diff ? rg[r].max_diff : rg[r].max_seed_diff;
        C.gaps |= rg[r].max_gapo > 0;
        C.wide |= bound > 14;
        C.nib_ok &= bound <= 6;
        C.max_entries = rg[r].max_entries > C.max_entries ? rg[r].max_entries : C.max_entries;
    }
    return C;
}

struct LaunchPlan {
    size_t lanes, blocks;
    uint32_t nt;
    uint32_t pcap, hcap, nb;
    bool gaps, wide;
    bool nib;
    uint32_t off_heads, off_wb, off_ws;
    uint32_t nib_wb, nib_ws;
    size_t lds;
    bool huge;
    uint32_t ntab;
    size_t resident;
    size_t res_lanes = 0;
};

enum { PASS_MAIN = 0, PASS_BIG = 1, PASS_HUGE = 2 };

static int plan_launch(hsa_index *ix, int n_jobs, int max_len, int max_seed, const RegimePlan &R, int mode,
                       LaunchPlan &P, uint32_t ent_bytes = 16)
{
    const int nb = R.nb, max_entries = R.max_entries;
    const bool gaps = R.gaps, wide = R.wide, nib_ok = R.nib_ok;
    const bool big = mode == PASS_BIG;
    P.huge = mode == PASS_HUGE;
    P.ntab = (uint32_t)ix->staged_ntab;
    P.nb = (uint32_t)nb;
    P.gaps = gaps;
    P.wide = wide;
    const uint32_t esz = wide ? 2u : 1u;
    P.nib = false;
    auto layout = [&](uint32_t nt) {
        const uint32_t epw = P.nib ? 8u : 4u / esz;
        P.nt = nt;
        P.off_heads = 2 * P.ntab + 128;
        P.off_wb = P.off_heads + (uint32_t)nb * nt * (P.huge ? 4u : 2u);
        P.nib_wb = ((uint32_t)max_len + 7u) / 8u;
        P.nib_ws = ((uint32_t)max_seed + 7u) / 8u;
        const uint32_t wbw = P.nib ? P.nib_wb : (uint32_t)max_len / epw + 1u;
        const uint32_t wsw = P.nib ? P.nib_ws : (uint32_t)max_seed / epw + 1u;
        P.off_ws = P.off_wb + wbw * nt * 4u;
        P.lds = ((size_t)P.off_ws + (size_t)wsw * nt * 4u + 15) / 16 * 16;
        int per_cu = (int)((160u * 1024u) / P.lds);
        const int cap = 4 * HSA_WAVES_SIMD / (int)(nt / 64);
        const int want = g_waves_per_cu / (int)(nt / 64);
        if (per_cu > cap) per_cu = cap;
        if (per_cu > want) per_cu = want > 0 ? want : 1;
        return per_cu;
    };
    static const int force256 = getenv("HSA_WG256") != nullptr;
    auto best = [&]() {
        int per_cu = layout(P.huge ? 64 : 256);
        if (per_cu < 4 && !force256 && !P.huge) {
            const int p64 = layout(64);
            if (p64 > per_cu * 4) per_cu = p64;
            else per_cu = layout(256);
        }
        return per_cu;
    };
    int per_cu = best();
    const char *wf = getenv("HSA_WFMT");
    const bool force_nib = wf && !strcmp(wf, "nib"), no_nib = wf && !strcmp(wf, "byte");
    if (nib_ok && !wide && !P.huge && !no_nib && (force_nib || (!gaps && per_cu * (int)(P.nt / 64) < 16))) {
        const int waves8 = per_cu * (int)(P.nt / 64);
        const LaunchPlan keep = P;
        P.nib = true;
        const int per_nib = best();
        if (!force_nib && per_nib * (int)(P.nt / 64) <= waves8) { P = keep; }
        else per_cu = per_nib;
    }
    if (P.lds > 160 * 1024) { hsa_set_error("reads too long for the LDS budget (%zu bytes)", P.lds); return HSA_E_ARG; }
    if (per_cu < 1) { hsa_set_error("search kernel does not fit (LDS %zu)", P.lds); return HSA_E_ARG; }
    const uint32_t NTB = P.nt;
    size_t blocks = (size_t)ix->n_cu * per_cu;
    P.resident = blocks * NTB;
    size_t need_blocks = ((size_t)n_jobs + NTB - 1) / NTB;
    if (P.huge) {
        blocks = 1;
    } else if (big) {
        static const size_t big_lanes = getenv("HSA_BIG_LANES") ? strtoull(getenv("HSA_BIG_LANES"), nullptr, 10) : 4096;
        const size_t big_blocks = big_lanes / NTB > 0 ? big_lanes / NTB : 1;
        blocks = need_blocks < big_blocks ? need_blocks : big_blocks;
        P.res_lanes = big_blocks * NTB;
    } else if (need_blocks < blocks) {
        blocks = need_blocks;
    }
    if (blocks < 1) blocks = 1;
    P.blocks = blocks;
    P.lanes = blocks * NTB;
    if (getenv("HSA_VERBOSE")) {
        int occ = 0;
        (void)hipOccupancyMaxActiveBlocksPerMultiprocessor(&occ, k_search<1, true, uint8_t, 256>, 256, P.lds);
        fprintf(stderr, "[hsa] launch: %d CUs x %d workgroups of %u lanes (runtime occupancy query says %d), "
                "LDS %zu B, %zu workgroups, %d buckets%s\n", ix->n_cu, per_cu, P.nt, occ, P.lds, blocks, nb,
                P.nib ? ", 4-bit rows" : "");
    }
    static const int pool_env = getenv("HSA_POOL_ENTRIES") ? atoi(getenv("HSA_POOL_ENTRIES")) : 0;
    const int pool_main = g_pool_entries ? g_pool_entries : pool_env > 0 && pool_env <= 65535 ? pool_env : 0;
    P.pcap = big ? 65535u : (uint32_t)(pool_main ? pool_main : (gaps ? (max_len <= 128 ? 16384 : 32768) : 8192));
    static const int pool_short = getenv("HSA_POOL_SHORT") ? atoi(getenv("HSA_POOL_SHORT")) : 8192;
    if (!big && !pool_main && max_len <= 32 && pool_short > 0 && pool_short <= 65535) P.pcap = (uint32_t)pool_short;
    P.hcap = big ? 16384u : (uint32_t)g_hit_cap;
    if (P.huge) {
        const uint64_t want = (uint64_t)(max_entries > 0 ? max_entries : 0) + 16u;
        P.pcap = (uint32_t)(want < (4ull << 20) ? want : (4ull << 20));
        P.hcap = 262144u;
    } else if (ent_bytes > 16 && !big) {
        const size_t budget = (size_t)64 << 30;
        if (P.lanes * P.pcap * ent_bytes > budget) {
            const size_t p = budget / (P.lanes * ent_bytes);
            P.pcap = (uint32_t)(p < 1024 ? 1024 : p);
        }
    }
    return 0;
}

template <typename WT, int NT, typename IT>
static void launch_search_nt(const LaunchPlan &P, const SearchArgs &A, hipStream_t st)
{
    const dim3 g((unsigned)P.blocks), b(NT);
    if (P.nb <= 32) {
        if (P.gaps) hipLaunchKernelGGL((k_search<0, true, WT, NT, false, IT>), g, b, P.lds, st, A);
        else hipLaunchKernelGGL((k_search<0, false, WT, NT, false, IT>), g, b, P.lds, st, A);
    } else if (P.nb <= 64) {
        if (P.gaps) hipLaunchKernelGGL((k_search<1, true, WT, NT, false, IT>), g, b, P.lds, st, A);
        else hipLaunchKernelGGL((k_search<1, false, WT, NT, false, IT>), g, b, P.lds, st, A);
    } else {
        if (P.gaps) hipLaunchKernelGGL((k_search<2, true, WT, NT, false, IT>), g, b, P.lds, st, A);
        else hipLaunchKernelGGL((k_search<2, false, WT, NT, false, IT>), g, b, P.lds, st, A);
    }
}

template <typename WT, typename IT>
static void launch_search(const LaunchPlan &P, const SearchArgs &A, hipStream_t st)
{
    if constexpr (!std::is_same<WT, WNib>::value) {
        if (P.nib) {
            if (P.nt == 64) launch_search_nt<WNib, 64, IT>(P, A, st);
            else launch_search_nt<WNib, 256, IT>(P, A, st);
            return;
        }
    }
    if (P.huge) {
        const dim3 g((unsigned)P.blocks), b(64);
        if (P.gaps) hipLaunchKernelGGL((k_search<2, true, WT, 64, true, IT>), g, b, P.lds, st, A);
        else hipLaunchKernelGGL((k_search<2, false, WT, 64, true, IT>), g, b, P.lds, st, A);
        return;
    }
    if (P.nt == 64) launch_search_nt<WT, 64, IT>(P, A, st);
    else launch_search_nt<WT, 256, IT>(P, A, st);
}

static uint32_t trie_levels(const hsa_index *ix, bool wide)
{
    const char *te = getenv("HSA_TRIE");
    return ix->trie_depth > 0 && ix->trie_wide == wide && !(te && atoi(te) == 0) ? ix->trie_depth : 0u;
}

struct MgPass {
    const hsa_mg_job_t *d_mg;
    int32_t *d_cw;
};

struct PassIO {
    const hsa_job_t *jobs;
    const int32_t *list;
    int n;
    const uint8_t *codes;
    int32_t *n_aln;
    uint32_t *flags;
    uint64_t *hit_off;
    uint32_t *hits;
    uint64_t hit_cap;
    unsigned long long *ctr;
    int max_len, max_seed;
    MgPass mg;
};

struct PassLink {
    int32_t *ovf_list = nullptr;
    const unsigned long long *n_dev = nullptr;
    uint32_t qctr = CTR_Q_MAIN;
    uint32_t ovf_ctr = CTR_OVF_MAIN;
};

template <typename IT = uint32_t>
static int pass_args(hsa_index *ix, const LaunchPlan &P, SearchScratch &S, const PassIO &io, const PassLink &lk,
                     SearchArgs &A)
{
    constexpr size_t WGB = sizeof(IT);
    const bool mg = io.mg.d_mg != nullptr;
    const uint32_t esz = P.wide ? 2u : 1u;
    const uint32_t rb = (((uint32_t)io.max_len + 1u) * esz + 3u) & ~3u, rs = (((uint32_t)io.max_seed + 1u) * esz + 3u) & ~3u;
    const uint32_t rg = (uint32_t)io.max_len + 1u;
    const size_t rows = ((size_t)io.n + 63) / 64 * 64 * 2;
    const size_t row_bytes = rb + rs + WGB * (size_t)rg + (mg ? 4 * (size_t)rg : 0);
    if (int rc = hsa_grow(&ix->d_wrows, &ix->d_wrows_cap, rows * row_bytes + 10 * (size_t)io.n + 1024)) return rc;
    uint8_t *wr = (uint8_t *)ix->d_wrows;
    A.fwd = RankDir{ix->blk[0], ix->isa0};
    A.rev = RankDir{ix->blk[1], ix->risa0};
    A.T = ix->T;
    memcpy(A.C, ix->C, sizeof A.C);
    A.fwd64 = hsa_rank_dir64(ix, 0);
    A.rev64 = hsa_rank_dir64(ix, 1);
    A.T64 = ix->T64;
    memcpy(A.C64, ix->C64, sizeof A.C64);
    A.regimes = (const hsa_regime_t *)ix->d_in; A.bmap = (const uint8_t *)ix->d_in + 256;
    A.jobs = io.jobs; A.job_list = io.list; A.n_jobs = io.n; A.codes = io.codes;
    A.n_aln = io.n_aln; A.flags = io.flags; A.hit_off = io.hit_off; A.hits = io.hits; A.hit_cap = io.hit_cap;
    A.ctr = io.ctr;
    A.wb = wr; A.ws = wr + rows * rb; A.wg = reinterpret_cast<uint32_t *>(wr + rows * (rb + rs));
    A.rb = rb; A.rs = rs; A.rg = rg;
    A.pool = S.pool; A.nxt = S.nxt; A.hbuf = S.hbuf;
    A.pcap = P.pcap; A.hcap = P.hcap;
    A.nb = P.nb; A.off_heads = P.off_heads; A.off_wb = P.off_wb; A.off_ws = P.off_ws;
    A.nib_wb = P.nib_wb; A.nib_ws = P.nib_ws;
    A.mm_buckets = ix->staged_mmb ? 1u : 0u;
    A.ntab = P.ntab;
    A.batch_k = (uint32_t)g_batch_k;
    A.batch_idle = (uint32_t)g_batch_idle;
    A.ovf_list = lk.ovf_list; A.n_dev = lk.n_dev; A.qctr = lk.qctr; A.ovf_ctr = lk.ovf_ctr;
    A.split = 0; A.sp_n = nullptr; A.sp_off = nullptr; A.sp_q = nullptr; A.sp_p = nullptr;
    A.ktd = trie_levels(ix, sizeof(IT) == 8);
    A.ktw = A.ktd ? ix->d_trie_w : nullptr;
    A.sdc = sizeof(IT) == 4 ? ix->sdepth : 0u;
    A.stw = A.sdc ? ix->d_trie_s : nullptr;
    A.wkey = nullptr; A.perm = nullptr; A.okey = 0;
    A.fwd_list = nullptr; A.fwd_n = nullptr; A.fwd_only = 0; A.rmap = nullptr;
    A.fr_budget = 0; A.fr_demand = 0; A.fr_cap = 0;
    A.fr_ent = nullptr; A.fr_tag = nullptr; A.fr_rq = nullptr; A.fr_st = nullptr; A.fr_q = nullptr; A.fr_p = nullptr; A.fr_c = nullptr;
    A.mg = io.mg.d_mg; A.cw = io.mg.d_cw;
    A.wbid = mg ? reinterpret_cast<int32_t *>(wr + rows * (rb + rs + WGB * (size_t)rg)) : nullptr;
    A.wq = reinterpret_cast<uint32_t *>(wr + rows * row_bytes);
    return 0;
}

static bool use_help()
{
    const char *e = getenv("HSA_HELP");
    return e && atoi(e) != 0;
}

template <typename IT>
static bool help_kernel(const LaunchPlan &P) { return use_help() && HSA_HELPERS && P.gaps && sizeof(IT) == 4; }

static bool use_split(const LaunchPlan &P, const PassIO &io, const PassLink &lk, bool help)
{
    if (io.mg.d_mg || lk.n_dev || lk.qctr != CTR_Q_MAIN || P.huge || io.n <= 0) return false;
    const char *e = getenv("HSA_SPLIT");
    if (e) return atoi(e) != 0;
    return (help ? (size_t)io.n : 2 * (size_t)io.n) <= P.resident;
}

template <typename IT>
static int help_args(hsa_index *ix, SearchArgs &A, size_t items, const LaunchPlan &P, hipStream_t st)
{
    if (!help_kernel<IT>(P) || ix->staged_min_entries <= (int)P.pcap + 16) return 0;
    auto env = [](const char *k, long d) { const char *v = getenv(k); return v ? atol(v) : d; };
    const long budget = env("HSA_HELP_BUDGET", 512), demand = env("HSA_HELP_DEMAND", (long)(P.lanes / 2));
    const long cap = env("HSA_HELP_CAP", 1l << 20);
    if (budget <= 0 || cap <= 0 || cap > (1l << 24) || demand < 0 || items >= (1u << 26)) return 0;
    auto al = [](size_t x) { return (x + 255) / 256 * 256; };
    const size_t o_st = 256, o_q = o_st + al(items * 4), o_p = o_q + al(items * 8), o_tag = o_p + al(items * 8);
    const size_t o_rq = o_tag + al((size_t)cap * 4);
    const size_t o_ent = o_rq + al((size_t)cap * 4), total = o_ent + (size_t)cap * FR_CH * FR_EW * 4;
    int rc = hsa_grow(&ix->d_help, &ix->d_help_cap, total);
    if (rc) return rc;
    char *d = (char *)ix->d_help;
    HSA_HIP(hipMemsetAsync(d, 0, o_ent, st));
    A.fr_budget = (uint32_t)budget; A.fr_demand = (uint32_t)demand; A.fr_cap = (uint32_t)cap;
    A.fr_c = (unsigned long long *)d;
    A.fr_st = (uint32_t *)(d + o_st);
    A.fr_q = (unsigned long long *)(d + o_q);
    A.fr_p = (unsigned long long *)(d + o_p);
    A.fr_tag = (uint32_t *)(d + o_tag);
    A.fr_rq = (uint32_t *)(d + o_rq);
    A.fr_ent = (uint32_t *)(d + o_ent);
    return 0;
}

static int scratch_fit(hsa_index *ix, SearchScratch &S, LaunchPlan &P, size_t EW)
{
    const size_t lb = P.huge ? 4 : 2, floor_cap = 512;
    auto pe_of = [&](uint32_t pc) { return (size_t)((pc + 31u) & ~31u) * EW; };
    const size_t rl = P.res_lanes > P.lanes ? P.res_lanes : P.lanes;
    auto bytes = [&](uint32_t pc) { return rl * (pe_of(pc) * (16 + lb) + (size_t)P.hcap * EW * 36); };
    const bool held = S.pool && lb == S.link_bytes && rl * pe_of(P.pcap) <= S.pool_entries &&
                      rl * (size_t)P.hcap * EW <= S.hit_entries;
    if (!held && !P.huge) {
        const char *cm = getenv("HSA_SCRATCH_MB");
        const size_t cap_mb = cm ? strtoull(cm, nullptr, 10) : 0;
        size_t fr = 0, tot = 0;
        if (hipMemGetInfo(&fr, &tot) != hipSuccess) { (void)hipGetLastError(); fr = (size_t)-1 / 2; }
        fr += S.pool_entries * (16 + S.link_bytes) + S.hit_entries * 36;
        size_t avail = fr > ((size_t)2 << 30) ? fr - ((size_t)2 << 30) : 0;
        if (cap_mb && avail > (cap_mb << 20)) avail = cap_mb << 20;
        const uint32_t want = P.pcap;
        while (bytes(P.pcap) > avail && P.pcap > floor_cap) P.pcap = P.pcap / 2 > floor_cap ? P.pcap / 2 : floor_cap;
        if (P.pcap != want && getenv("HSA_VERBOSE"))
            fprintf(stderr, "[hsa] search scratch: pool %u -> %u entries per lane (%.1f GB for %zu lanes; %.1f GB "
                            "available)\n", want, P.pcap, bytes(P.pcap) / 1e9, P.lanes, avail / 1e9);
    }
    for (;;) {
        const int rc = hsa_scratch_reserve(S, rl, pe_of(P.pcap), (size_t)P.hcap * EW, lb);
        if (rc != HSA_E_MEM || P.huge || P.pcap <= floor_cap) return rc;
        P.pcap = P.pcap / 2 > floor_cap ? P.pcap / 2 : floor_cap;
        if (getenv("HSA_VERBOSE")) fprintf(stderr, "[hsa] search scratch: allocation failed, pool -> %u per lane\n", P.pcap);
    }
}

template <typename IT = uint32_t>
static int launch_pass(hsa_index *ix, const LaunchPlan &P0, SearchScratch &S, const PassIO &io, const PassLink &lk,
                       hipStream_t st)
{
    const int n = io.n;
    const bool mg = io.mg.d_mg != nullptr;
    const bool first = lk.qctr == CTR_Q_MAIN;
    const bool split = use_split(P0, io, lk, help_kernel<IT>(P0));
    LaunchPlan P = P0;
    if (split) {
        const size_t need = (2 * (size_t)n + P.nt - 1) / P.nt, cap = P.resident / P.nt;
        P.blocks = need < cap ? need : cap;
        P.lanes = P.blocks * P.nt;
    }
    constexpr size_t EW = sizeof(IT) / 4;
    int rc = scratch_fit(ix, S, P, EW);
    if (rc) return rc;
    SearchArgs A;
    if (mg) {
        if constexpr (sizeof(IT) != 4) {
            hsa_set_error("caller-width searches (bwt_match_gap) take 32-bit indexes");
            return HSA_E_ARG;
        } else {
            if ((rc = pass_args<IT>(ix, P, S, io, lk, A))) return rc;
            if (first) HSA_HIP(hipMemsetAsync(io.ctr, 0, CTR_SLOTS * sizeof(unsigned long long), st));
            const unsigned nb = (unsigned)(((size_t)n + BLOCK - 1) / BLOCK);
            if (P.wide) hipLaunchKernelGGL(k_widths_import<uint16_t>, dim3(nb ? nb : 1), dim3(BLOCK), 0, st, A);
            else hipLaunchKernelGGL(k_widths_import<uint8_t>, dim3(nb ? nb : 1), dim3(BLOCK), 0, st, A);
            HSA_HIP(hipGetLastError());
            if (ix->ev_split) HSA_HIP(hipEventRecord(ix->ev_split, st));
            if (P.wide) launch_search<uint16_t, uint32_t>(P, A, st);
            else launch_search<uint8_t, uint32_t>(P, A, st);
            HSA_HIP(hipGetLastError());
            hipLaunchKernelGGL(k_widths_export, dim3(nb ? nb : 1), dim3(BLOCK), 0, st, A);
            HSA_HIP(hipGetLastError());
            return 0;
        }
    }
    if ((rc = pass_args<IT>(ix, P, S, io, lk, A))) return rc;
    if (split) {
        const size_t m = 2 * (size_t)n, al = (m * 8 + 255) / 256 * 256;
        if ((rc = hsa_grow(&ix->d_split, &ix->d_split_cap, 3 * al))) return rc;
        char *d = (char *)ix->d_split;
        A.split = 1;
        A.sp_off = (uint64_t *)d;
        A.sp_n = (int32_t *)(d + al);
        A.sp_q = (uint32_t *)(d + al + al / 2);
        A.sp_p = (uint32_t *)(d + 2 * al);
        if (!P.huge && (rc = help_args<IT>(ix, A, m, P, st))) return rc;
    }
    if (first) HSA_HIP(hipMemsetAsync(io.ctr, 0, CTR_SLOTS * sizeof(unsigned long long), st));
    const char *oe = getenv("HSA_ORDER");
    const bool order = !split && !lk.n_dev && first && n > 0 &&
                       (oe ? atoi(oe) != 0 : (size_t)n > P.resident);
    uint32_t *d_oh = nullptr;
    if (order) {
        char *tail = (char *)A.wq + 4 * (size_t)n;
        A.wkey = (uint8_t *)tail;
        static const uint32_t okey = getenv("HSA_ORDER_KEY") ? (uint32_t)atoi(getenv("HSA_ORDER_KEY")) : 1u;
        A.okey = okey;
        const size_t ko = (2 * (size_t)n + 15) / 16 * 16;
        d_oh = (uint32_t *)(tail + ko);
        HSA_HIP(hipMemsetAsync(d_oh, 0, 32 * 4, st));
    }
    const char *le = getenv("HSA_LAZY");
    const bool lazy = !split && !lk.n_dev && first && n > 0 && (le ? atoi(le) != 0 : io.max_len >= 200);
    unsigned long long *d_fwd_n = nullptr;
    int32_t *d_list2 = nullptr;
    unsigned long long *d_n2 = nullptr;
    if (lazy) {
        if ((rc = hsa_grow(&ix->d_fwd, &ix->d_fwd_cap, 512 + 12 * (size_t)n))) return rc;
        d_fwd_n = (unsigned long long *)ix->d_fwd;
        d_n2 = d_fwd_n + 1;
        HSA_HIP(hipMemsetAsync(d_fwd_n, 0, 16, st));
        A.fwd_n = d_fwd_n;
        A.fwd_list = (int32_t *)((char *)ix->d_fwd + 128);
        d_list2 = A.fwd_list + ((size_t)n + 31) / 32 * 32;
        A.rmap = d_list2 + ((size_t)n + 31) / 32 * 32;
    }
    if (lazy) {
        const unsigned rblocks = (unsigned)(((size_t)n + BLOCK - 1) / BLOCK);
        if (P.wide) {
            hipLaunchKernelGGL((k_widths_reads<uint16_t, IT>), dim3(rblocks), dim3(BLOCK), 0, st, A, 1u, d_list2, d_n2);
            hipLaunchKernelGGL((k_widths_reads<uint16_t, IT>), dim3(rblocks), dim3(BLOCK), 0, st, A, 3u, d_list2, d_n2);
        } else {
            hipLaunchKernelGGL((k_widths_reads<uint8_t, IT>), dim3(rblocks), dim3(BLOCK), 0, st, A, 1u, d_list2, d_n2);
            hipLaunchKernelGGL((k_widths_reads<uint8_t, IT>), dim3(rblocks), dim3(BLOCK), 0, st, A, 3u, d_list2, d_n2);
        }
    } else {
        size_t wblocks = ((size_t)n * 2 + BLOCK - 1) / BLOCK;
        if (wblocks < 1) wblocks = 1;
        if (P.wide) hipLaunchKernelGGL((k_widths<uint16_t, IT>), dim3((unsigned)wblocks), dim3(BLOCK), 0, st, A);
        else hipLaunchKernelGGL((k_widths<uint8_t, IT>), dim3((unsigned)wblocks), dim3(BLOCK), 0, st, A);
    }
    HSA_HIP(hipGetLastError());
    if (order) {
        int32_t *d_perm = (int32_t *)(d_oh + 32);
        const unsigned nb = (unsigned)(((size_t)n + BLOCK - 1) / BLOCK);
        hipLaunchKernelGGL(k_order_hist, dim3(nb), dim3(BLOCK), 0, st, A, d_oh);
        hipLaunchKernelGGL(k_order_scan, dim3(1), dim3(1), 0, st, d_oh);
        hipLaunchKernelGGL(k_order_scatter, dim3(nb), dim3(BLOCK), 0, st, A, d_oh, d_perm);
        HSA_HIP(hipGetLastError());
        A.perm = d_perm;
    }
    if (ix->ev_split && first) HSA_HIP(hipEventRecord(ix->ev_split, st));
    if (P.wide) launch_search<uint16_t, IT>(P, A, st);
    else launch_search<uint8_t, IT>(P, A, st);
    HSA_HIP(hipGetLastError());
    if (lazy) {
        SearchArgs F = A;
        F.job_list = A.fwd_list; F.n_dev = d_fwd_n; F.qctr = CTR_Q_FWD; F.fwd_only = 1;
        F.fwd_list = nullptr; F.fwd_n = nullptr; F.wkey = nullptr; F.perm = nullptr; F.rmap = nullptr;
        const unsigned rblocks = (unsigned)(((size_t)n + BLOCK - 1) / BLOCK);
        if (P.wide) hipLaunchKernelGGL((k_widths_reads<uint16_t, IT>), dim3(rblocks), dim3(BLOCK), 0, st, F, 2u, d_list2, d_n2);
        else hipLaunchKernelGGL((k_widths_reads<uint8_t, IT>), dim3(rblocks), dim3(BLOCK), 0, st, F, 2u, d_list2, d_n2);
        HSA_HIP(hipGetLastError());
        if (P.wide) launch_search<uint16_t, IT>(P, F, st);
        else launch_search<uint8_t, IT>(P, F, st);
        HSA_HIP(hipGetLastError());
    }
    if (split) {
        const unsigned nb = (unsigned)(((size_t)n + BLOCK - 1) / BLOCK);
        hipLaunchKernelGGL(k_split_finalize, dim3(nb), dim3(BLOCK), 0, st, A);
        HSA_HIP(hipGetLastError());
        if (getenv("HSA_VERBOSE")) {
            fprintf(stderr, "[hsa] strand-split main pass: %d reads on %zu lanes\n", n, P.lanes);
            if (A.fr_c) {
                unsigned long long c[9];
                HSA_HIP(hipMemcpyAsync(c, A.fr_c, sizeof c, hipMemcpyDeviceToHost, st));
                HSA_HIP(hipStreamSynchronize(st));
                fprintf(stderr, "[hsa] helpers: %llu offers (%llu refused), %llu chunks, %llu sub-searches, %llu strands "
                                "answered by them, %llu rank queries in sub-searches\n", c[4], c[5], c[0], c[6], c[7], c[8]);
            }
        }
    }
    return 0;
}

static int jobs_limits(const hsa_job_t *jobs, int n, int &max_len, int &max_seed)
{
    max_len = 0; max_seed = 0;
    for (int j = 0; j < n; ++j) {
        if (jobs[j].len > ANY_MAX_LEN) { hsa_set_error("read %d longer than %d (gap_entry_t.info, bwtgap.c:157)", j, ANY_MAX_LEN); return HSA_E_ARG; }
        if (jobs[j].max_diff < -1) { hsa_set_error("max_diff out of range"); return HSA_E_ARG; }
        if ((int)jobs[j].len > max_len) max_len = (int)jobs[j].len;
        if ((int)jobs[j].len > jobs[j].seed_len && jobs[j].seed_len > max_seed) max_seed = jobs[j].seed_len;
    }
    return 0;
}

static int stage_regimes(hsa_index *ix, const hsa_regime_t *regimes, int n_regimes, int &nb, hipStream_t st,
                         bool force = false)
{
    void *before = ix->d_in;
    if (int rc = hsa_grow(&ix->d_in, &ix->d_in_cap, 1536)) return rc;
    force = force || before != ix->d_in;
    static_assert(256 + 2 * MAXS <= sizeof(ix->staged), "staging copy");
    uint8_t host[256 + 2 * MAXS];
    memset(host, 0xFF, sizeof host);
    memcpy(host, regimes, sizeof(hsa_regime_t) * n_regimes);
    nb = 1;
    int ntab = 8;
    for (int r = 0; r < n_regimes; ++r) {
        int k = bucket_map(regimes[r], host + 256 + r * MAXS);
        nb = k > nb ? k : nb;
        ntab = regimes[r].n_stacks > ntab ? regimes[r].n_stacks : ntab;
    }
    if (nb > MAXB) { hsa_set_error("%d reachable scores: at most %d stack buckets", nb, MAXB); return HSA_E_ARG; }
    ix->staged_ntab = (ntab + 7) / 8 * 8;
    ix->staged_mmb = mm_buckets(regimes, n_regimes, host + 256);
    ix->staged_min_entries = regimes[0].max_entries;
    for (int r = 1; r < n_regimes; ++r)
        if (regimes[r].max_entries < ix->staged_min_entries) ix->staged_min_entries = regimes[r].max_entries;
    if (!force && ix->staged_valid && memcmp(ix->staged, host, sizeof host) == 0) return 0;
    memcpy(ix->staged, host, sizeof host);
    ix->staged_valid = 1;
    HSA_HIP(hipMemcpyAsync(ix->d_in, ix->staged, sizeof host, hipMemcpyHostToDevice, st));
    HSA_HIP(hipStreamSynchronize(st));
    return 0;
}

template <typename IT = uint32_t>
static int run_capacity_passes(hsa_index *ix, const RegimePlan &C, const PassIO &io, PassLink main, bool zero_ctr,
                               hipEvent_t ev_split, hipStream_t st)
{
    constexpr uint32_t EB = 4u * sizeof(IT);
    LaunchPlan P, B, H;
    int rc;
    if ((rc = plan_launch(ix, io.n, io.max_len, io.max_seed, C, PASS_MAIN, P, EB)) ||
        (rc = plan_launch(ix, io.n, io.max_len, io.max_seed, C, PASS_BIG, B, EB)) ||
        (rc = plan_launch(ix, io.n, io.max_len, io.max_seed, C, PASS_HUGE, H, EB)))
        return rc;
    if ((rc = hsa_grow(&ix->d_ovf, &ix->d_ovf_cap, (size_t)io.n * 4 + 64)) ||
        (rc = hsa_grow(&ix->d_ovf2, &ix->d_ovf2_cap, (size_t)io.n * 4 + 64)))
        return rc;
    if (zero_ctr) HSA_HIP(hipMemsetAsync(io.ctr, 0, CTR_SLOTS * sizeof(unsigned long long), st));
    int32_t *const ovf = (int32_t *)ix->d_ovf, *const ovf2 = (int32_t *)ix->d_ovf2;
    main.ovf_list = ovf;
    const PassLink big{.ovf_list = ovf2, .n_dev = io.ctr + CTR_OVF_MAIN, .qctr = CTR_Q_BIG, .ovf_ctr = CTR_OVF_BIG};
    const PassLink huge{.ovf_list = nullptr, .n_dev = io.ctr + CTR_OVF_BIG, .qctr = CTR_Q_HUGE};
    PassIO io_b = io, io_h = io;
    io_b.list = ovf; io_h.list = ovf2;
    if (ev_split) ix->ev_split = ev_split;
    rc = launch_pass<IT>(ix, P, ix->main, io, main, st);
    if (!rc) rc = launch_pass<IT>(ix, B, ix->big, io_b, big, st);
    if (!rc) rc = launch_pass<IT>(ix, H, ix->huge, io_h, huge, st);
    ix->ev_split = ix->evm;
    return rc;
}

enum {
    ANY_N_FAST = 0,
    ANY_N_ANY = 1,
    ANY_Q = 2,
    ANY_N_OVF = 3,
    ANY_Q_BIG = 4
};

struct AnyBufs {
    hsa_regime_t *reg;
    unsigned long long *cnt;
    int32_t *l_fast, *l_any, *l_ovf;
    const hsa_regime_t *regimes;
    int n_regimes;
};

static int any_prepare(hsa_index *ix, const hsa_regime_t *regimes, int n_regimes, size_t n, hipStream_t st, AnyBufs &B)
{
    const size_t lb = (n * 4 + 255) / 256 * 256;
    if (ix->d_any_cap > ((size_t)8 << 30)) {
        HSA_HIP(hipStreamSynchronize(st));
        (void)hipFree(ix->d_any);
        ix->d_any = nullptr;
        ix->d_any_cap = 0;
    }
    int rc = hsa_grow(&ix->d_any_aux, &ix->d_any_aux_cap, 512 + 3 * lb);
    if (rc) return rc;
    char *d = (char *)ix->d_any_aux;
    B.reg = (hsa_regime_t *)d;
    B.cnt = (unsigned long long *)(d + 256);
    B.l_fast = (int32_t *)(d + 512);
    B.l_any = (int32_t *)(d + 512 + lb);
    B.l_ovf = (int32_t *)(d + 512 + 2 * lb);
    B.regimes = regimes;
    B.n_regimes = n_regimes;
    HSA_HIP(hipMemcpyAsync(B.reg, regimes, sizeof(hsa_regime_t) * n_regimes, hipMemcpyHostToDevice, st));
    HSA_HIP(hipMemsetAsync(B.cnt, 0, 64, st));
    HSA_HIP(hipStreamSynchronize(st));
    return 0;
}

template <typename IT>
static int any_pass(hsa_index *ix, const AnyBufs &B, const PassIO &io, const unsigned long long *n_dev, bool big,
                    hipStream_t st)
{
    const uint32_t max_len = (uint32_t)io.max_len, max_seed = (uint32_t)io.max_seed;
    size_t n_bound = (size_t)io.n;
    if (n_bound == 0) return 0;
    if (big && n_dev) {
        unsigned long long cnt = 0;
        HSA_HIP(hipMemcpyAsync(&cnt, n_dev, sizeof cnt, hipMemcpyDeviceToHost, st));
        HSA_HIP(hipStreamSynchronize(st));
        if (cnt == 0) return 0;
        n_bound = (size_t)cnt;
    }
    AnyArgs A;
    memset(&A, 0, sizeof A);
    A.fwd = RankDir{ix->blk[0], ix->isa0};
    A.rev = RankDir{ix->blk[1], ix->risa0};
    A.fwd64 = hsa_rank_dir64(ix, 0);
    A.rev64 = hsa_rank_dir64(ix, 1);
    A.T = ix->T; A.T64 = ix->T64;
    memcpy(A.C, ix->C, sizeof A.C);
    memcpy(A.C64, ix->C64, sizeof A.C64);
    A.regimes = B.reg; A.jobs = io.jobs; A.list = io.list; A.n_dev = n_dev; A.n_host = n_dev ? 0 : io.n;
    A.codes = io.codes;
    A.mg = io.mg.d_mg; A.cw = io.mg.d_cw;
    A.n_aln = io.n_aln; A.flags = io.flags; A.hit_off = io.hit_off; A.hits = io.hits; A.hit_cap = io.hit_cap;
    A.ctr = io.ctr;
    A.qhead = B.cnt + (big ? ANY_Q_BIG : ANY_Q);
    A.ovf_list = big ? nullptr : B.l_ovf;
    A.ovf_n = big ? nullptr : B.cnt + ANY_N_OVF;
    uint32_t nst = 1, max_entries = 0;
    for (int r = 0; r < B.n_regimes; ++r) {
        nst = (uint32_t)B.regimes[r].n_stacks > nst ? (uint32_t)B.regimes[r].n_stacks : nst;
        max_entries = (uint32_t)B.regimes[r].max_entries > max_entries ? (uint32_t)B.regimes[r].max_entries : max_entries;
    }
    const uint64_t want = (uint64_t)max_entries + 16u;
    static const uint32_t pcap1 = getenv("HSA_ANY_PCAP") ? (uint32_t)atoi(getenv("HSA_ANY_PCAP")) : 8192u;
    const uint32_t pcap = big ? (uint32_t)(want < (4ull << 20) ? want : (4ull << 20)) : pcap1;
    const uint32_t hcap = big ? 262144u : 512u;
    const size_t lb = any_layout<IT>(A, max_len, max_seed, nst, pcap, hcap, 10);
    size_t budget = (size_t)4 << 30, lanes_max = 16384;
    if (big) {
        size_t fr = 0, tot = 0;
        HSA_HIP(hipMemGetInfo(&fr, &tot));
        budget = fr / 2 < ((size_t)64 << 30) ? fr / 2 : ((size_t)64 << 30);
        lanes_max = 4096;
    }
    size_t lanes = n_bound < lanes_max ? n_bound : lanes_max;
    if (lanes * lb > budget) lanes = budget / lb;
    if (lanes < 1) lanes = 1;
    A.nlanes = (uint32_t)lanes;
    if (lanes * lb + 256 > ix->d_any_cap) HSA_HIP(hipStreamSynchronize(st));
    int rc = hsa_grow(&ix->d_any, &ix->d_any_cap, lanes * lb + 256);
    if (rc) return rc;
    A.scratch = (uint8_t *)ix->d_any;
    if (getenv("HSA_VERBOSE"))
        fprintf(stderr, "[hsa] k_search_any%s: %zu lanes x %zu B (pool %u, hits %u, %u stacks, reads <= %u bp)\n",
                big ? " (large pass)" : "", lanes, lb, pcap, hcap, nst, max_len);
    hipLaunchKernelGGL(k_search_any<IT>, dim3((unsigned)((lanes + 63) / 64)), dim3(64), 0, st, A);
    HSA_HIP(hipGetLastError());
    return 0;
}

template <typename IT>
static int any_passes(hsa_index *ix, const AnyBufs &B, const PassIO &io, const unsigned long long *n_dev, hipStream_t st)
{
    PassIO big = io;
    big.list = B.l_ovf;
    const int rc = any_pass<IT>(ix, B, io, n_dev, false, st);
    return rc ? rc : any_pass<IT>(ix, B, big, B.cnt + ANY_N_OVF, true, st);
}

template <typename IT>
static int search_device_impl(hsa_index_t *ix, const hsa_regime_t *regimes, int n_regimes, const hsa_device_batch_t *b,
                              void *stream)
{
    if (n_regimes < 1 || n_regimes > 2) { hsa_set_error("1 or 2 regimes"); return HSA_E_ARG; }
    if (sizeof(IT) == 8 && !ix->wide) { hsa_set_error("not a 64-bit index (hsa_index_create_device64)"); return HSA_E_ARG; }
    int rc = check_regimes(regimes, n_regimes);
    if (rc) return rc;
    if (b->max_len < 1 || b->max_len > ANY_MAX_LEN || b->max_seed < 0 || b->max_seed > ANY_MAX_LEN) {
        hsa_set_error("max_len/max_seed out of range");
        return HSA_E_ARG;
    }
    HSA_HIP(hipSetDevice(ix->device));
    hipStream_t st = stream ? (hipStream_t)stream : ix->stream;
    hipEvent_t *pe = ix->pev[ix->pev_n % hsa_index::PASS_RING];
    for (int j = 0; j < 3; ++j)
        if (!pe[j]) HSA_HIP(hipEventCreate(&pe[j]));
    const bool fast_rg = fast_regimes(regimes, n_regimes);
    const bool any_path = !fast_rg || (uint32_t)b->max_len > FAST_MAX_LEN;
    AnyBufs AB{};
// ... 36 lines not shown
```

### hsa_amd/csrc/hsa_splice_prefetch.h

```cpp
#pragma once

static size_t al(size_t x) { return (x + 255) / 256 * 256; }

struct SeedArgs {
    RankDir rev;
    uint32_t T;
    uint32_t C[5];
    const hsa_job_t *rjobs;
    const uint8_t *rcodes;
    const uint32_t *rflags;
    uint32_t n_reads;
    int32_t max_seed_diff;
    uint32_t code_stride, pair_stride;
    hsa_job_t *jobs;
    hsa_mg_job_t *mg;
    uint8_t *codes;
    int32_t *cw;
    int32_t *list;
    unsigned long long *count;
    unsigned long long *ctr;
};

__global__ void __launch_bounds__(BLOCK) k_seed_prep(SeedArgs a)
{
    const uint32_t t = blockIdx.x * BLOCK + threadIdx.x;
    const uint32_t r = t >> 1, s = t & 1u;
    if (r >= a.n_reads || !(a.rflags[r] & HSA_F_FALLBACK)) return;
    const hsa_job_t R = a.rjobs[r];
    const uint32_t L = R.len, sl = L / 3u;
    if (sl < 1) return;
    const uint32_t la2 = sl + L % 3u;
    auto base = [&](uint32_t p) -> uint32_t {
        const uint32_t c = a.rcodes[R.off + (s ? L - 1u - p : p)];
        return s && c < 4 ? 3u - c : c;
    };
    uint32_t coff[3], poff[3], la[3];
    {
        uint32_t co = 0, po = 0;
        for (uint32_t i = 0; i < 6; ++i) {
            const uint32_t l_i = sl + (i % 3 == 2 ? L % 3u : 0u);
            if (i / 3 == s) { coff[i % 3] = co; poff[i % 3] = po; la[i % 3] = l_i; }
            co += l_i; po += l_i + 1;
        }
    }
    uint8_t *const cbase = a.codes + (size_t)r * a.code_stride;
    int32_t *const wbase = a.cw + 2 * (size_t)r * a.pair_stride;
    uint32_t k = 0, l = a.T, bid = 0, bid_sl = 0, q = 0;
    for (uint32_t p = 0; p < la2; ++p) {
        const uint32_t c = base(p);
        if (c < 4) {
            uint32_t ok, ol;
            hsa_occ1_pair(a.rev, k, l + 1u, c, ok, ol);
            q += 2;
            const uint32_t cc = hsa_sel4(c, a.C[0], a.C[1], a.C[2], a.C[3]);
            k = cc + ok + 1u;
            l = cc + ol;
        }
        if (k > l || c > 3) { k = 0; l = a.T; ++bid; }
        const int32_t w = (int32_t)(l - k + 1u);
        for (uint32_t tt = 0; tt < 3; ++tt)
            if (p < la[tt]) { wbase[2 * (poff[tt] + p)] = w; wbase[2 * (poff[tt] + p) + 1] = (int32_t)bid; }
        if (p + 1 == sl) bid_sl = bid;
    }
    for (uint32_t tt = 0; tt < 3; ++tt) {
        const uint32_t term_bid = (la[tt] == sl ? bid_sl : bid) + 1u;
        wbase[2 * (poff[tt] + la[tt])] = 0;
        wbase[2 * (poff[tt] + la[tt]) + 1] = (int32_t)term_bid;
        for (uint32_t p = 0; p < la[tt]; ++p) cbase[coff[tt] + p] = (uint8_t)base(tt * sl + p);
        const uint32_t j = r * 6u + 3u * s + tt;
        hsa_job_t J;
        J.off = (uint64_t)r * a.code_stride + coff[tt];
        J.len = la[tt];
        J.max_diff = a.max_seed_diff;
        J.seed_len = (int32_t)la[tt];
        J.regime = 0;
        a.jobs[j] = J;
        hsa_mg_job_t M;
        M.wb_off = (uint64_t)r * a.pair_stride + poff[tt];
        M.ws_off = 0;
        M.strand = (int32_t)s;
        M.seed = HSA_SEED_ALIAS;
        a.mg[j] = M;
    }
    const unsigned long long b0 = atomicAdd(a.count, 3ull);
    for (uint32_t tt = 0; tt < 3; ++tt) a.list[b0 + tt] = (int32_t)(r * 6u + 3u * s + tt);
    atomicAdd(&a.ctr[CTR_WIDTH_Q], (unsigned long long)q);
}

extern "C" int hsa_splice_seeds_device(hsa_index_t *ix, const hsa_regime_t *seed_regime, const hsa_seed_batch_t *b,
                                       void *stream)
{
    if (int rc0 = hsa_need32(ix)) return rc0;
    int rc = check_regimes(seed_regime, 1);
    if (rc) return rc;
    if (seed_regime->max_gapo != 0) { hsa_set_error("seed searches have no gap opens (bwtgap.c:772)"); return HSA_E_ARG; }
    if (b->max_len < 3 || b->max_len > 1023 || b->n_jobs < 0) { hsa_set_error("max_len/n_jobs out of range"); return HSA_E_ARG; }
    const size_t n = (size_t)b->n_jobs, calls = 6 * n;
    if (n == 0) return 0;
    HSA_HIP(hipSetDevice(ix->device));
    hipStream_t st = stream ? (hipStream_t)stream : ix->stream;
    const uint32_t code_stride = (uint32_t)(2 * b->max_len), pair_stride = (uint32_t)(2 * b->max_len + 6);
    const size_t o_mg = al(calls * sizeof(hsa_job_t)), o_list = o_mg + al(calls * sizeof(hsa_mg_job_t));
    const size_t o_fl = o_list + al(calls * 4), o_cnt = o_fl + al(calls * 4), o_codes = o_cnt + 256;
    const size_t o_cw = o_codes + al(n * code_stride), total = o_cw + n * pair_stride * 8 + 256;
    if ((rc = hsa_grow(&ix->d_seed, &ix->d_seed_cap, total))) return rc;
    char *d = (char *)ix->d_seed;
    unsigned long long *cnt = (unsigned long long *)(d + o_cnt);
    unsigned long long *ctr = (unsigned long long *)b->d_counters;
    HSA_HIP(hipMemsetAsync(cnt, 0, 8, st));
    SeedArgs S;
    S.rev = RankDir{ix->blk[1], ix->risa0};
    S.T = ix->T;
    memcpy(S.C, ix->C, sizeof S.C);
    S.rjobs = b->d_jobs; S.rcodes = b->d_codes; S.rflags = b->d_flags; S.n_reads = (uint32_t)n;
    S.max_seed_diff = seed_regime->max_diff;
    S.code_stride = code_stride; S.pair_stride = pair_stride;
    S.jobs = (hsa_job_t *)d; S.mg = (hsa_mg_job_t *)(d + o_mg); S.codes = (uint8_t *)(d + o_codes);
    S.cw = (int32_t *)(d + o_cw); S.list = (int32_t *)(d + o_list); S.count = cnt; S.ctr = ctr;
    RegimePlan C = regime_plan(seed_regime, 1);
    C.nib_ok = false;
    if ((rc = stage_regimes(ix, seed_regime, 1, C.nb, st))) return rc;
    HSA_HIP(hipMemsetAsync(ctr, 0, CTR_SLOTS * sizeof(unsigned long long), st));
    hipLaunchKernelGGL(k_seed_prep, dim3((unsigned)((2 * n + BLOCK - 1) / BLOCK)), dim3(BLOCK), 0, st, S);
    HSA_HIP(hipGetLastError());
    HSA_HIP(hipEventRecord(ix->ev0, st));
    const PassIO io{.jobs = S.jobs, .list = S.list, .n = (int)calls, .codes = S.codes, .n_aln = b->d_n_aln,
                    .flags = (uint32_t *)(d + o_fl), .hit_off = b->d_hit_off, .hits = b->d_hits, .hit_cap = b->hit_cap,
                    .ctr = ctr, .max_len = b->max_len / 3 + 2, .max_seed = 0, .mg = {S.mg, S.cw}};
    if ((rc = run_capacity_passes(ix, C, io, PassLink{.n_dev = cnt, .qctr = CTR_Q_MG}, false, nullptr, st))) return rc;
    HSA_HIP(hipEventRecord(ix->ev1, st));
    return 0;
}

struct PfArgs {
    RankDir fwd, rev;
    uint32_t T;
    uint32_t C[5];
    uint32_t n, max_len, sc, rs, cws;
    const uint32_t *lens;
    const uint64_t *offs;
    const uint8_t *codes;
    const int32_t *amd;
    int32_t seed_max_diff;
    uint8_t *scodes;
    int32_t *rows;
    hsa_job_t *jobs;
    hsa_mg_job_t *mg;
    int32_t *cw;
    int32_t *list;
    int32_t *call_n;
    uint32_t *call_fl;
    unsigned long long *acount;
    const unsigned long long *d_n;
    uint64_t cwd;
    uint32_t prefix;
    const void *ktw;
    uint32_t ktd;
};

__device__ __forceinline__ uint32_t pf_n(const PfArgs &a) { return a.d_n ? (uint32_t)*a.d_n : a.n; }

__global__ void __launch_bounds__(BLOCK) k_pf_rows(PfArgs a)
{
    const uint32_t t = blockIdx.x * BLOCK + threadIdx.x;
    const uint32_t r = t / 6u, s = (t % 6u) & 1u, kind = (t % 6u) >> 1;
    if (r >= pf_n(a)) return;
    const uint32_t L = a.lens[r];
    const uint64_t off = a.offs[r];
    int32_t *const o = a.rows + 2 * ((size_t)r * 6u + kind * 2u + s) * a.rs;
    uint32_t k = 0, l = a.T, bid = 0;
    uint32_t cq = 0xFFFFFFFFu, cword = 0;
    auto base = [&](uint32_t p) -> uint32_t {
        const uint64_t ix = off + (s ? L - 1u - p : p);
        if ((uint32_t)(ix >> 2) != cq) {
            cword = *reinterpret_cast<const uint32_t *>(a.codes + (ix & ~(uint64_t)3));
            cq = (uint32_t)(ix >> 2);
        }
        const uint32_t c = (cword >> (((uint32_t)ix & 3u) * 8u)) & 0xFFu;
        return s && c < 4 ? 3u - c : c;
    };
    if (kind == 0 || kind == 1) {
        if (kind == 1 && L < 12u) return;
        const uint32_t p0 = kind == 1 ? L - 12u : 0u, n = kind == 1 ? 12u : L;
        uint8_t *const sc = a.scodes + (size_t)(2u * r + s) * a.sc;
        uint32_t tl = 0, tix = 0;
        for (uint32_t i = 0; i < n; ++i) {
            const uint32_t c = base(p0 + i);
            if (kind == 0) sc[i] = (uint8_t)c;
            if (c < 4) {
                if (tl < a.ktd) {
                    tix = tix * 4u + c;
                    ++tl;
                    trie_w_load<uint32_t>(a.ktw, trie_base(tl) + tix, k, l);
                } else {
                    uint32_t ok, ol;
                    hsa_occ1_pair(a.rev, k, l + 1u, c, ok, ol);
                    const uint32_t cc = hsa_sel4(c, a.C[0], a.C[1], a.C[2], a.C[3]);
                    k = cc + ok + 1u;
                    l = cc + ol;
                }
            }
            if (k > l || c > 3) { k = 0; l = a.T; ++bid; tl = 0; tix = 0; }
            *reinterpret_cast<int2 *>(o + 2 * i) = make_int2((int32_t)(l - k + 1u), (int32_t)bid);
        }
        *reinterpret_cast<int2 *>(o + 2 * n) = make_int2(0, (int32_t)(bid + 1u));
        return;
    }
    *reinterpret_cast<int2 *>(o) = make_int2(0, 0);
    for (uint32_t i = L - 1u; i > 0 && L > 0; --i) {
        const uint32_t c = base(i);
        if (c < 4) {
            uint32_t ok, ol;
            hsa_occ1_pair(a.fwd, k, l + 1u, c, ok, ol);
            const uint32_t cc = hsa_sel4(c, a.C[0], a.C[1], a.C[2], a.C[3]);
            k = cc + ok + 1u;
            l = cc + ol;
        }
        if (k > l || c > 3) { k = 0; l = a.T; ++bid; }
        *reinterpret_cast<int2 *>(o + 2 * i) = make_int2((int32_t)(l - k + 1u), (int32_t)bid);
    }
    *reinterpret_cast<int2 *>(o + 2 * L) = make_int2(0, (int32_t)(bid + 1u));
}

__global__ void __launch_bounds__(BLOCK) k_pf_seeds(PfArgs a)
{
    const uint32_t t = blockIdx.x * BLOCK + threadIdx.x;
    const uint32_t r = t / 6u, i = t % 6u, s = i / 3u, tt = i % 3u;
    if (r >= pf_n(a)) return;
    const uint32_t L = a.lens[r], sl = L / 3u, la = sl + (tt == 2u ? L % 3u : 0u);
    const uint32_t call = 8u * r + i;
    a.list[6u * r + i] = (int32_t)call;
    const int32_t *const w1 = a.rows + 2 * ((size_t)r * 6u + s) * a.rs;
    hsa_mg_job_t M;
    if (a.prefix) {
        M.wb_off = ((uint64_t)r * 6u + s) * a.rs;
        M.ws_off = HSA_MG_PREFIX;
    } else {
        int32_t *const cw = a.cw + 2 * (size_t)call * a.cws;
        for (uint32_t p = 0; p < la; ++p) { cw[2 * p] = w1[2 * p]; cw[2 * p + 1] = w1[2 * p + 1]; }
        cw[2 * la] = 0;
        cw[2 * la + 1] = (la ? w1[2 * (la - 1u) + 1] : 0) + 1;
        M.wb_off = a.cwd + (uint64_t)call * a.cws;
        M.ws_off = 0;
    }
    hsa_job_t J;
    J.off = (uint64_t)(2u * r + s) * a.sc + tt * sl;
    J.len = la;
    J.max_diff = a.seed_max_diff;
    J.seed_len = (int32_t)la;
    J.regime = 0;
    a.jobs[call] = J;
    M.strand = (int32_t)s;
    M.seed = HSA_SEED_ALIAS;
    a.mg[call] = M;
}

__global__ void __launch_bounds__(BLOCK) k_pf_anchors(PfArgs a)
{
    const uint32_t t = blockIdx.x * BLOCK + threadIdx.x;
    const uint32_t r = t >> 1, s = t & 1u;
    if (r >= pf_n(a)) return;
    const uint32_t L = a.lens[r], call = 8u * r + 6u + s;
    const int32_t *const cn = a.call_n + 8u * r + 3u * s;
    const uint32_t *const cf = a.call_fl + 8u * r + 3u * s;
    const bool done = !(cf[0] & HSA_F_OVERFLOW) && !(cf[1] & HSA_F_OVERFLOW) && !(cf[2] & HSA_F_OVERFLOW);
    const uint32_t mask = (cn[0] > 0) | (cn[1] > 0) << 1 | (cn[2] > 0) << 2;
    if (L <= 12u || !done || (mask != 3u && mask != 6u)) { a.call_n[call] = -1; return; }
    const bool tail = mask == 3u;
    const int32_t *const src = a.rows + 2 * ((size_t)r * 6u + (tail ? 2u : 0u) + s) * a.rs;
    int32_t *const cw = a.cw + 2 * (size_t)call * a.cws;
    for (uint32_t p = 0; p < 13u; ++p) { cw[2 * p] = src[2 * p]; cw[2 * p + 1] = src[2 * p + 1]; }
    hsa_job_t J;
    J.off = (uint64_t)(2u * r + s) * a.sc + (tail ? L - 12u : 0u);
// ... 45 lines not shown
    unsigned long long o = a.call_sa[c];
    for (int x = 0; x < n; ++x) {
        const uint32_t k = h[9 * x + 1], m = pf_sa_span(k, h[9 * x + 2]);
        for (uint32_t j = 0; j < m; ++j) a.idx[o++] = k + j;
    }
}

__global__ void __launch_bounds__(BLOCK) k_sp_prep(const hsa_job_t *jobs, const uint32_t *flags, const int32_t *n_aln,
                                                   uint32_t n, uint32_t max_len, uint32_t *res, uint32_t *lens,
                                                   uint64_t *offs, int32_t *amd, int32_t *idx, unsigned long long *cnt)
{
    const uint32_t j = blockIdx.x * BLOCK + threadIdx.x;
    if (j >= n || !(flags[j] & HSA_F_FALLBACK) || n_aln[j] != 0) return;
    const hsa_job_t J = jobs[j];
    if (J.len < 3u || J.len > max_len) {
        res[(size_t)j * HSA_SP_RES_WORDS] = HSA_SP_WIN;
        res[(size_t)j * HSA_SP_RES_WORDS + 1] = 0u;
        return;
    }
    const uint32_t r = (uint32_t)atomicAdd(cnt, 1ull);
    lens[r] = J.len;
    offs[r] = J.off;
    amd[r] = J.max_diff;
    idx[r] = (int32_t)j;
}

__global__ void k_sp_calls(const unsigned long long *cnt, unsigned long long *scnt) { *scnt = 6ull * *cnt; }

__global__ void k_sp_stats(const unsigned long long *cnt, const unsigned long long *ctr_s,
                           const unsigned long long *ctr_a, unsigned long long *out)
{
    out[0] = *cnt;
    out[5] = ctr_s[CTR_RANK] + ctr_s[CTR_WIDTH_Q] + ctr_a[CTR_RANK] + ctr_a[CTR_WIDTH_Q];
    out[6] = ctr_s[CTR_HITS] + ctr_a[CTR_HITS];
}

static PfArgs pf_args(const hsa_index *ix, uint32_t n, uint32_t M, int32_t seed_max_diff)
{
    PfArgs A;
    A.fwd = RankDir{ix->blk[0], ix->isa0};
    A.rev = RankDir{ix->blk[1], ix->risa0};
    A.T = ix->T;
    memcpy(A.C, ix->C, sizeof A.C);
    A.n = n; A.max_len = M; A.sc = (M + 15u) / 16u * 16u + 16u; A.rs = M + 1u; A.cws = M / 3u + 3u > 13u ? M / 3u + 3u : 13u;
    A.seed_max_diff = seed_max_diff;
    A.ktd = trie_levels(ix, false);
    A.ktw = A.ktd ? ix->d_trie_w : nullptr;
    return A;
}

enum PfCtr {
    PFC_SEED = 0,
    PFC_ANCHOR = PFC_SEED + CTR_SLOTS,
    PFC_N_ANCHOR = PFC_ANCHOR + CTR_SLOTS,
    PFC_SA_TOTAL,
    PFC_N_SEED,
    PFC_N_READS,
    PFC_SPLICE = 40,
    PFC_SLOTS = 128
};

enum : unsigned { PF_CODES = 1, PF_IDX = 2, PF_CALL_SA = 4, PF_RES = 8 };
struct PfLayout {
    unsigned opt;
    uint64_t cap_s, cap_a;
    size_t lens, offs, amd, idx, codes, sc, jobs, mg, list, ctr;
    size_t call_n, call_fl, call_hit, call_sa, rows, cw, hits_s, hits_a;
    size_t res, total;
    bool device_batch() const { return opt & PF_IDX; }
};

static PfLayout pf_layout(size_t N, size_t codes_len, const PfArgs &A, unsigned opt)
{
    PfLayout L;
    const size_t calls = 8 * N;
    size_t o = 0;
    const auto region = [&o](size_t bytes) { const size_t at = o; o += al(bytes); return at; };
    L.opt = opt; L.cap_s = 6 * N * 16 + 65536; L.cap_a = 2 * N * 16 + 16384;
    L.lens = region(N * 4); L.offs = region(N * 8); L.amd = region(N * 4);
    L.idx = region(opt & PF_IDX ? N * 4 : 0); L.codes = region(opt & PF_CODES ? codes_len + 64 : 0);
    L.sc = region(2 * N * A.sc + 64);
    L.jobs = region(calls * sizeof(hsa_job_t)); L.mg = region(calls * sizeof(hsa_mg_job_t)); L.list = region(calls * 4);
    L.ctr = region(PFC_SLOTS * sizeof(unsigned long long));
    L.call_n = region(calls * 4); L.call_fl = region(calls * 4); L.call_hit = region(calls * 8);
    L.call_sa = region(opt & PF_CALL_SA ? calls * 8 : 0);
    L.rows = region(N * 6 * A.rs * 8); L.cw = region(calls * A.cws * 8);
    L.hits_s = region(L.cap_s * 36); L.hits_a = region(L.cap_a * 36);
    L.res = region(opt & PF_RES ? N * HSA_SP_RES_WORDS * 4 : 0);
    L.total = o + 256;
    return L;
}

struct PfSearch {
    PfArgs A;
    PfLayout L;
    const hsa_regime_t *seed_rg, *anchor_rg;
    hipStream_t st;
    char *d;
    unsigned long long *ctr;
    int nb;
    bool wide;
    template <class T> T *at(size_t region) const { return (T *)(d + region); }
};

static int pf_check(const hsa_index *ix, const hsa_regime_t *seed_rg, const hsa_regime_t *anchor_rg, bool args_ok,
                    const char *entry)
{
    if (int rc = hsa_need32(ix)) return rc;
    if (!seed_rg || !anchor_rg || !args_ok) { hsa_set_error("%s: null argument", entry); return HSA_E_ARG; }
    const hsa_regime_t rg2[2] = {*seed_rg, *anchor_rg};
    if (int rc = check_regimes(rg2, 2)) return rc;
    if (seed_rg->max_gapo != 0) { hsa_set_error("seed searches have no gap opens (bwtgap.c:772)"); return HSA_E_ARG; }
    if (!fast_regimes(rg2, 2)) { hsa_set_error("%s: options outside k_search's layouts", entry); return HSA_E_ARG; }
    return 0;
}

static int pf_bind(hsa_index *ix, PfSearch &F, const uint8_t *codes, bool prefix)
{
    const PfLayout &L = F.L;
    PfArgs &A = F.A;
    if (int rc = hsa_grow(&ix->d_pf, &ix->d_pf_cap, L.total)) return rc;
    F.d = (char *)ix->d_pf;
    F.ctr = F.at<unsigned long long>(L.ctr);
    HSA_HIP(hipMemsetAsync(F.ctr, 0, PFC_SLOTS * sizeof(unsigned long long), F.st));
    A.lens = F.at<uint32_t>(L.lens); A.offs = F.at<uint64_t>(L.offs); A.amd = F.at<int32_t>(L.amd);
    A.codes = codes ? codes : F.at<uint8_t>(L.codes);
    A.scodes = F.at<uint8_t>(L.sc); A.rows = F.at<int32_t>(L.rows); A.cw = F.at<int32_t>(L.cw);
    A.jobs = F.at<hsa_job_t>(L.jobs); A.mg = F.at<hsa_mg_job_t>(L.mg); A.list = F.at<int32_t>(L.list);
    A.call_n = F.at<int32_t>(L.call_n); A.call_fl = F.at<uint32_t>(L.call_fl);
    A.acount = F.ctr + PFC_N_ANCHOR;
    A.d_n = L.device_batch() ? F.ctr + PFC_N_READS : nullptr;
    A.cwd = (L.cw - L.rows) / 8;
    A.prefix = prefix ? 1u : 0u;
    return 0;
}

static PfDev pf_dev(const PfSearch &F)
{
    const PfArgs &A = F.A;
    PfDev pd;
    pd.n = A.n; pd.max_len = A.max_len; pd.sc = A.sc; pd.rs = A.rs; pd.cws = A.cws;
    pd.lens = A.lens; pd.amd = A.amd; pd.scodes = A.scodes; pd.rows = A.rows; pd.cw = A.cw;
    pd.call_n = A.call_n; pd.call_fl = A.call_fl; pd.call_hit = F.at<uint64_t>(F.L.call_hit);
    pd.hits_s = F.at<uint32_t>(F.L.hits_s); pd.hits_a = F.at<uint32_t>(F.L.hits_a);
    pd.d_n = A.d_n; pd.idx = F.L.device_batch() ? F.at<int32_t>(F.L.idx) : nullptr;
    return pd;
}

static int pf_passes(hsa_index *ix, const PfSearch &F, bool anchors, int n_upper)
{
    const PfArgs &A = F.A;
    const PfLayout &L = F.L;
    RegimePlan C = regime_plan(anchors ? F.anchor_rg : F.seed_rg, 1);
    C.nb = F.nb; C.wide = F.wide; C.nib_ok = false;
    const PassIO io{.jobs = A.jobs, .list = A.list + (anchors ? 6 * (size_t)A.n : 0), .n = n_upper, .codes = A.scodes,
                    .n_aln = A.call_n, .flags = A.call_fl, .hit_off = F.at<uint64_t>(L.call_hit),
                    .hits = F.at<uint32_t>(anchors ? L.hits_a : L.hits_s), .hit_cap = anchors ? L.cap_a : L.cap_s,
                    .ctr = F.ctr + (anchors ? PFC_ANCHOR : PFC_SEED), .max_len = anchors ? 12 : (int)(A.max_len / 3u + 2u),
                    .max_seed = 0, .mg = {A.mg, A.rows}};
    const PassLink link{.n_dev = F.ctr + (anchors ? PFC_N_ANCHOR : PFC_N_SEED), .qctr = CTR_Q_MG};
    return run_capacity_passes(ix, C, io, link, true, nullptr, F.st);
}

static int pf_run(hsa_index *ix, PfSearch &F)
{
    const size_t N = F.A.n;
    const bool host = !F.L.device_batch();
    hipStream_t st = F.st;
    const unsigned grid6 = (unsigned)((6 * N + BLOCK - 1) / BLOCK), grid2 = (unsigned)((2 * N + BLOCK - 1) / BLOCK);
    HSA_HIP(hipMemsetAsync(F.A.scodes, 4, 2 * N * F.A.sc + 64, st));
    hipLaunchKernelGGL(k_pf_rows, dim3(grid6), dim3(BLOCK), 0, st, F.A);
    hipLaunchKernelGGL(k_pf_seeds, dim3(grid6), dim3(BLOCK), 0, st, F.A);
    HSA_HIP(hipGetLastError());
    const hsa_regime_t rg2[2] = {*F.seed_rg, *F.anchor_rg};
    F.nb = 0; F.wide = regime_plan(rg2, 2).wide;
    if (int rc = stage_regimes(ix, rg2, 2, F.nb, st)) return rc;
    const unsigned long long n_seed = 6 * N;
    unsigned long long n_anchor = 2 * N;
    if (host) {
        HSA_HIP(hipMemcpyAsync(F.ctr + PFC_N_SEED, &n_seed, 8, hipMemcpyHostToDevice, st));
        HSA_HIP(hipEventRecord(ix->ev0, st));
    }
    if (int rc = pf_passes(ix, F, false, (int)n_seed)) return rc;
    hipLaunchKernelGGL(k_pf_anchors, dim3(grid2), dim3(BLOCK), 0, st, F.A);
    HSA_HIP(hipGetLastError());
    if (host) {
        HSA_HIP(hipMemcpyAsync(&n_anchor, F.ctr + PFC_N_ANCHOR, 8, hipMemcpyDeviceToHost, st));
        HSA_HIP(hipStreamSynchronize(st));
    }
    return n_anchor ? pf_passes(ix, F, true, (int)n_anchor) : 0;
}

static int pf_host_splice(hsa_index *ix, const PfSearch &F, const hsa_regime_t &ext_rg, uint32_t *res,
                          hsa_splice_pf_t *out, hsa_splice_stats_t *sst)
{
    const PfArgs &A = F.A;
    hipStream_t st = F.st;
    uint32_t *d_res = F.at<uint32_t>(F.L.res);
    HSA_HIP(hipEventRecord(ix->ev1, st));
    if (int rc = hsa_splice_device_launch(ix, pf_dev(F), ext_rg, d_res, F.ctr + PFC_SPLICE, st)) return rc;
    HSA_HIP(hipEventRecord(ix->ev_sp, st));
    HSA_HIP(hipMemcpyAsync(res, d_res, (size_t)A.n * HSA_SP_RES_WORDS * 4, hipMemcpyDeviceToHost, st));
    unsigned long long sc4[4];
    HSA_HIP(hipMemcpyAsync(sc4, F.ctr + PFC_SPLICE, sizeof sc4, hipMemcpyDeviceToHost, st));
    HSA_HIP(hipStreamSynchronize(st));
    float ms = 0, sms = 0;
    HSA_HIP(hipEventElapsedTime(&ms, ix->ev0, ix->ev1));
    HSA_HIP(hipEventElapsedTime(&sms, ix->ev1, ix->ev_sp));
    out->n = (int)A.n; out->max_len = (int)A.max_len; out->row_stride = (int)A.rs; out->cw_stride = (int)A.cws;
    out->kernel_ms = ms;
    if (sst) {
        sst->kernel_ms = sms;
        sst->extensions = sc4[0]; sst->pops = sc4[1]; sst->sa_lookups = sc4[2]; sst->not_answered = sc4[3];
    }
    return 0;
}

static int pf_host_tables(hsa_index *ix, const PfSearch &F, hsa_splice_pf_t *out, double t0)
{
    const PfArgs &A = F.A;
    const PfLayout &L = F.L;
    hipStream_t st = F.st;
    const size_t calls = 8 * (size_t)A.n;
    const unsigned grid = (unsigned)((calls + BLOCK - 1) / BLOCK);
    const uint32_t *d_hs = F.at<uint32_t>(L.hits_s), *d_ha = F.at<uint32_t>(L.hits_a);
    PfSaArgs S;
    S.n_calls = (uint32_t)calls;
    S.call_n = A.call_n; S.call_hit = F.at<uint64_t>(L.call_hit);
    S.hits_s = d_hs; S.hits_a = d_ha;
    S.call_sa = F.at<unsigned long long>(L.call_sa); S.total = F.ctr + PFC_SA_TOTAL; S.idx = nullptr;
    const bool with_sa = ix->d_sa != nullptr;
    if (with_sa) hipLaunchKernelGGL(k_pf_sa, dim3(grid), dim3(BLOCK), 0, st, S, 0);
    HSA_HIP(hipGetLastError());
    unsigned long long hc[PFC_SPLICE];
    HSA_HIP(hipMemcpyAsync(hc, F.ctr, sizeof hc, hipMemcpyDeviceToHost, st));
    HSA_HIP(hipStreamSynchronize(st));
    const uint64_t n_sa = with_sa ? hc[PFC_SA_TOTAL] : 0;
    if (int rc = n_sa ? hsa_grow(&ix->d_pf2, &ix->d_pf2_cap, al(n_sa * 4) + n_sa * 16 + 256) : 0) return rc;
    uint32_t *d_idx = (uint32_t *)ix->d_pf2, *d_sao = (uint32_t *)((char *)ix->d_pf2 + al(n_sa * 4));
    if (n_sa) {
        S.idx = d_idx;
        hipLaunchKernelGGL(k_pf_sa, dim3(grid), dim3(BLOCK), 0, st, S, 1);
        HSA_HIP(hipGetLastError());
        if (int rc = hsa_sa_position_device(ix, n_sa, d_idx, d_sao, st)) return rc;
    }
    HSA_HIP(hipEventRecord(ix->ev1, st));
    const auto q = [&L](size_t region) { return region - L.call_n; };
    const uint64_t nh_s = hc[PFC_SEED + CTR_HITS] < L.cap_s ? hc[PFC_SEED + CTR_HITS] : L.cap_s;
    const uint64_t nh_a = hc[PFC_ANCHOR + CTR_HITS] < L.cap_a ? hc[PFC_ANCHOR + CTR_HITS] : L.cap_a;
    const size_t h_hits = q(L.hits_s), h_need = h_hits + (nh_s + nh_a) * 36 + al(n_sa * 16) + 256;
    if (h_need > ix->h_pf_cap) {
        if (ix->h_pf) (void)hipHostFree(ix->h_pf);
        ix->h_pf = nullptr; ix->h_pf_cap = 0;
        const size_t want = h_need + h_need / 4 > ((size_t)64 << 20) ? h_need + h_need / 4 : ((size_t)64 << 20);
        HSA_HIP(hipHostMalloc(&ix->h_pf, want, hipHostMallocDefault));
        ix->h_pf_cap = want;
    }
    char *h = (char *)ix->h_pf;
    HSA_HIP(hipMemcpyAsync(h, F.d + L.call_n, h_hits + nh_s * 36, hipMemcpyDeviceToHost, st));
    if (nh_a) HSA_HIP(hipMemcpyAsync(h + h_hits + nh_s * 36, d_ha, nh_a * 36, hipMemcpyDeviceToHost, st));
    const size_t h_sa = al(h_hits + (nh_s + nh_a) * 36);
    if (n_sa) HSA_HIP(hipMemcpyAsync(h + h_sa, d_sao, n_sa * 16, hipMemcpyDeviceToHost, st));
    HSA_HIP(hipStreamSynchronize(st));
    float ms = 0;
    HSA_HIP(hipEventElapsedTime(&ms, ix->ev0, ix->ev1));
    int32_t *cn = (int32_t *)h;
    const uint32_t *cf = (const uint32_t *)(h + q(L.call_fl));
    uint64_t *ch = (uint64_t *)(h + q(L.call_hit));
    for (size_t c = 0; c < calls; ++c) {
        if ((c & 7u) >= 6u && cn[c] >= 0) ch[c] += nh_s;
        if (cn[c] >= 0 && (cf[c] & HSA_F_OVERFLOW)) cn[c] = -2;
    }
    out->n = (int)A.n; out->max_len = (int)A.max_len; out->row_stride = (int)A.rs; out->cw_stride = (int)A.cws;
    out->call_n = cn; out->call_hit = ch;
    out->call_sa = with_sa ? (const uint64_t *)(h + q(L.call_sa)) : nullptr;
    out->rows = (const int32_t *)(h + q(L.rows));
    out->wafter = (const int32_t *)(h + q(L.cw));
    out->hits = (const uint32_t *)(h + h_hits);
    out->sa = n_sa ? (const uint32_t *)(h + h_sa) : nullptr;
    out->n_hits = nh_s + nh_a; out->n_sa = n_sa;
    out->kernel_ms = ms;
    if (getenv("HSA_VERBOSE")) {
        struct timespec t; clock_gettime(CLOCK_MONOTONIC, &t);
        fprintf(stderr, "[hsa] splice prefetch on the device: %u reads, %llu seed + %llu anchor calls, %llu hits, %llu SA "
                        "lookups, %.1f ms (kernels %.1f ms)\n", A.n, 6ull * A.n, hc[PFC_N_ANCHOR],
                (unsigned long long)(nh_s + nh_a), (unsigned long long)n_sa, 1e3 * (t.tv_sec + 1e-9 * t.tv_nsec - t0), ms);
    }
    return 0;
}

static int pf_batch(hsa_index_t *ix, const hsa_regime_t *seed_rg, const hsa_regime_t *anchor_rg, int n,
                    const uint32_t *lens, const uint64_t *offs, const uint8_t *codes, size_t codes_len,
                    const int32_t *anchor_max_diff, hsa_splice_pf_t *out, const hsa_regime_t *ext_rg, uint32_t *res,
                    hsa_splice_stats_t *sst)
{
    memset(out, 0, sizeof *out);
    if (sst) memset(sst, 0, sizeof *sst);
    if (n <= 0) return 0;
    int rc = pf_check(ix, seed_rg, anchor_rg, lens && offs && codes && anchor_max_diff,
                      ext_rg ? "hsa_splice_match_batch" : "hsa_splice_prefetch_batch");
    if (rc) return rc;
    uint32_t M = 0;
    for (int r = 0; r < n; ++r) {
        if (lens[r] < 3 || lens[r] > 3 * (FAST_MAX_LEN - 2)) {
            hsa_set_error("splice prefetch: read %d of %u bases", r, lens[r]);
            return HSA_E_ARG;
        }
// ... 70 lines not shown
```

Baseline: 58.99 million.

## Add mixed-format search with 4-bit seed rows and register-aware occupancy planning

Adds a mixed layout where the main width row stays 8-bit but the seed width row is stored at 4 bits per entry. This shrinks the per-lane LDS footprint so more workgroups fit per CU when the seed diff bound allows it. Launch planning now reads the kernel's register count to cap waves per SIMD. It also raises the default waves-per-CU target and always tries 64-lane workgroups. Kernel dispatch is consolidated into a function-pointer selector, and the new template instantiations add compile time and code size.

Measured after the change: 61.42 million, median of 6. 1.04x the previous value.

```diff
diff --git a/hsa_amd/csrc/hsa_index.hip b/hsa_amd/csrc/hsa_index.hip
--- a/hsa_amd/csrc/hsa_index.hip
+++ b/hsa_amd/csrc/hsa_index.hip
@@ -12,7 +12,7 @@
 #include "hsa_trie.h"
 
 static thread_local char g_err[1024] = "";
-int g_waves_per_cu = 16;
+int g_waves_per_cu = 32;
 int g_pool_entries = 0;
 int g_batch_k = getenv("HSA_BATCH_K") ? atoi(getenv("HSA_BATCH_K")) : 32;
 int g_batch_idle = getenv("HSA_BATCH_IDLE") ? atoi(getenv("HSA_BATCH_IDLE")) : 768;
diff --git a/hsa_amd/csrc/hsa_search.hip b/hsa_amd/csrc/hsa_search.hip
--- a/hsa_amd/csrc/hsa_search.hip
+++ b/hsa_amd/csrc/hsa_search.hip
@@ -288,6 +288,7 @@
     RegimePlan R = regime_plan(regimes, n_regimes);
     R.nb = H.nb;
     R.nib_ok = R.nib_ok && !mh;
+    R.snib_ok = R.snib_ok && !mh;
     for (int j = 0; j < n_jobs && R.nib_ok; ++j) R.nib_ok = jobs[j].max_diff <= 6;
     if ((rc = plan_launch(ix, n_jobs, max_len, max_seed, R, PASS_MAIN, P))) return rc;
     HSA_HIP(hipEventRecord(ix->ev0, st));
diff --git a/hsa_amd/csrc/hsa_search_kernels.h b/hsa_amd/csrc/hsa_search_kernels.h
--- a/hsa_amd/csrc/hsa_search_kernels.h
+++ b/hsa_amd/csrc/hsa_search_kernels.h
@@ -45,7 +45,7 @@
     uint32_t *hbuf;
     uint32_t pcap, hcap, nb;
     uint32_t off_heads, off_wb, off_ws;
-    uint32_t nib_wb, nib_ws;
+    uint32_t lds_wb, lds_ws;
     uint32_t mm_buckets;
     int32_t *ovf_list;
     const unsigned long long *n_dev;
@@ -248,6 +248,8 @@
     static constexpr uint32_t BIDB = 3u, BIDM = 7u, EQ = 8u, EB = 4u, EPW = 8u;
 };
 
+template <typename WT, bool SN> using SeedFmt = WFmt<typename std::conditional<SN, WNib, WT>::type>;
+
 __device__ __forceinline__ uint32_t nib4(uint32_t x)
 {
     uint32_t b = x & 0x0F0F0F0Fu;
@@ -322,7 +324,7 @@
     return (uint8_t)(b << 4 | (w.tail < 16u ? 2u : w.tail < 48u ? 1u : 0u));
 }
 
-template <typename WT, typename IT>
+template <typename WT, typename IT, bool SN = false>
 __device__ __forceinline__ WRow width_row(const SearchArgs &a, uint32_t R, uint32_t strand, const hsa_job_t &J)
 {
     using F = WFmt<WT>;
@@ -361,7 +363,8 @@
         width_step<WT, IT>(a, f, t, len, cf, t < len ? F::code_bits(cf) : 0u, brow, wrow, st_q, st_b, st_t);
         if (has_seed && t <= slen) {
             const uint32_t cs = t < slen ? base(s0 + t, 1) : 4u;
-            width_step<WT, IT>(a, sd, t, slen, cs, 0u, srow, nullptr, st_q, st_b, st_t);
+            width_step<typename std::conditional<SN, WNib, WT>::type, IT>(a, sd, t, slen, cs, 0u, srow, nullptr, st_q,
+                                                                          st_b, st_t);
         }
     }
     return WRow{st_q, st_b, st_t, f.bid, len - f.lr};
@@ -376,7 +379,7 @@
 #define HSA_NOFWD 0xFFFFFFFFu
 #define HSA_F_NEEDFWD 0x100u
 
-template <typename WT, typename IT = uint32_t>
+template <typename WT, typename IT = uint32_t, bool SN = false>
 __global__ void __launch_bounds__(BLOCK) k_widths(SearchArgs a)
 {
     const uint32_t R = blockIdx.x * BLOCK + threadIdx.x;
@@ -385,7 +388,7 @@
     WRow w{0, 0, 0, 0};
     if (R < 2u * n_jobs) {
         const hsa_job_t J = a.jobs[a.job_list ? a.job_list[q] : (int)q];
-        w = width_row<WT, IT>(a, R, strand, J);
+        w = width_row<WT, IT, SN>(a, R, strand, J);
         if (!strand) a.wq[q] = w.q;
         if (a.wkey) a.wkey[R] = cost_key(a, w);
     }
@@ -396,7 +399,7 @@
     wave_add(&a.ctr[CTR_TRIE], w.t);
 }
 
-template <typename WT, typename IT = uint32_t>
+template <typename WT, typename IT = uint32_t, bool SN = false>
 __global__ void __launch_bounds__(BLOCK) k_widths_reads(SearchArgs a, uint32_t mode, int32_t *list2,
                                                         unsigned long long *n2)
 {
@@ -408,7 +411,7 @@
         const uint32_t q = mode == 3 ? (uint32_t)list2[p] : p;
         const hsa_job_t J = a.jobs[a.job_list ? a.job_list[q] : (int)q];
         const uint32_t R = mode == 1 ? q : mode == 3 ? (uint32_t)(((uint32_t)a.n_jobs + 63u) & ~63u) + p : 2u * q;
-        w = width_row<WT, IT>(a, R, mode == 1 ? 1u : 0u, J);
+        w = width_row<WT, IT, SN>(a, R, mode == 1 ? 1u : 0u, J);
         if (mode == 3) a.rmap[q] = (int32_t)R;
         const uint8_t key = cost_key(a, w);
         if (mode == 1) {
@@ -576,10 +579,12 @@
     }
 }
 
-template <int MW, bool GAPS, typename WT, int NT, bool HUGE = false, typename IT = uint32_t>
+template <int MW, bool GAPS, typename WT, int NT, bool HUGE = false, typename IT = uint32_t, bool SN = false>
 __global__ void __launch_bounds__(NT, HSA_WAVES_SIMD) k_search(SearchArgs a)
 {
     using F = WFmt<WT>;
+    using FS = SeedFmt<WT, SN>;
+    static_assert(!SN || (std::is_same<WT, uint8_t>::value && !HUGE), "mixed format: 8-bit rows, not the HUGE pass");
     using E = Ent<IT>;
     using CT = typename std::conditional<sizeof(IT) == 8, int64_t, int>::type;
     constexpr uint32_t HW = HitW<IT>::STAGE, OW = HitW<IT>::OUT;
@@ -668,7 +673,7 @@
         else return WB(p);
     };
     auto wsg = [&](int p) -> uint32_t {
-        if constexpr (F::NIB) return (s_ns[((uint32_t)p >> 3) * NT + tid] >> (((uint32_t)p & 7u) * 4u)) & 15u;
+        if constexpr (FS::NIB) return (s_ns[((uint32_t)p >> 3) * NT + tid] >> (((uint32_t)p & 7u) * 4u)) & 15u;
         else return WS(p);
     };
     auto wbs = [&](int p, uint32_t v) {
@@ -757,17 +762,18 @@
                         if (j + u < nn) dst[(j + u) * NT + tid] = nib4(w[2u * u]) | nib4(w[2u * u + 1u]) << 16;
                 }
             };
-            pack(src, nwb, s_nb, r->nib_wb);
+            pack(src, nwb, s_nb, r->lds_wb);
             if (C_SEED(ctl) && !C_ALIAS(ctl))
-                pack(reinterpret_cast<const uint32_t *>(r->ws) + row_base(r->rs / 4), r->rs / 4, s_ns, r->nib_ws);
+                pack(reinterpret_cast<const uint32_t *>(r->ws) + row_base(r->rs / 4), r->rs / 4, s_ns, r->lds_ws);
         } else {
         uint32_t *const db = reinterpret_cast<uint32_t *>(s_wb) + (tid & ~63u);
-        for (uint32_t q = 0; q < nwb; ++q)
+        const uint32_t lwb = SN ? r->lds_wb : nwb;
+        for (uint32_t q = 0; q < lwb; ++q)
             __builtin_amdgcn_global_load_lds(src + q * 64, db + q * NT, 4, 0, 0);
         if (C_SEED(ctl) && !C_ALIAS(ctl)) {
             const uint32_t *ss = reinterpret_cast<const uint32_t *>(r->ws) + row_base(r->rs / 4);
             uint32_t *const ds = reinterpret_cast<uint32_t *>(s_ws) + (tid & ~63u);
-            const uint32_t nws = r->rs / 4;
+            const uint32_t nws = SN ? r->lds_ws : r->rs / 4;
             for (uint32_t q = 0; q < nws; ++q)
                 __builtin_amdgcn_global_load_lds(ss + q * 64, ds + q * NT, 4, 0, 0);
         }
@@ -1382,11 +1388,12 @@
                 if (C_SEED(ctl) && ii > 0) {
                     int ems = RG(max_seed_diff) - (emm + ego);
                     if (R_MODE & MODE_GAPE) ems -= ege;
-                    const uint32_t s1 = C_ALIAS(ctl) ? wbg(ii - 1) : wsg(ii - 1);
-                    const uint32_t s0 = C_ALIAS(ctl) ? wbg(ii) : wsg(ii);
-                    const int c1 = (int)(s1 & F::BIDM), c0 = (int)(s0 & F::BIDM);
+                    const bool alias = !SN && C_ALIAS(ctl);
+                    const uint32_t s1 = alias ? wbg(ii - 1) : wsg(ii - 1);
+                    const uint32_t s0 = alias ? wbg(ii) : wsg(ii);
+                    const int c1 = (int)(s1 & FS::BIDM), c0 = (int)(s0 & FS::BIDM);
                     if (c1 > ems - 1) allow_diff = 0;
-                    else if (c1 == ems - 1 && c0 == ems - 1 && (s1 & F::EQ)) allow_M = 0;
+                    else if (c1 == ems - 1 && c0 == ems - 1 && (s1 & FS::EQ)) allow_M = 0;
                 }
             }
             const uint32_t sc = F::NIB ? cur_c : getc(i);
diff --git a/hsa_amd/csrc/hsa_search_launch.h b/hsa_amd/csrc/hsa_search_launch.h
--- a/hsa_amd/csrc/hsa_search_launch.h
+++ b/hsa_amd/csrc/hsa_search_launch.h
@@ -1,4 +1,7 @@
 #pragma once
+#include <map>
+#include <mutex>
+
 #include "hsa_search_kernels.h"
 
 static int check_regimes(const hsa_regime_t *rg, int n)
@@ -63,18 +66,19 @@
 
 struct RegimePlan {
     int nb;
-    bool gaps, wide, nib_ok;
+    bool gaps, wide, nib_ok, snib_ok;
     int max_entries;
 };
 
 static RegimePlan regime_plan(const hsa_regime_t *rg, int n)
 {
-    RegimePlan C{.nb = 0, .gaps = false, .wide = false, .nib_ok = true, .max_entries = 0};
+    RegimePlan C{.nb = 0, .gaps = false, .wide = false, .nib_ok = true, .snib_ok = true, .max_entries = 0};
     for (int r = 0; r < n; ++r) {
         const int bound = rg[r].max_diff > rg[r].max_seed_diff ? rg[r].max_diff : rg[r].max_seed_diff;
         C.gaps |= rg[r].max_gapo > 0;
         C.wide |= bound > 14;
         C.nib_ok &= bound <= 6;
+        C.snib_ok &= rg[r].max_seed_diff <= 6;
         C.max_entries = rg[r].max_entries > C.max_entries ? rg[r].max_entries : C.max_entries;
     }
     return C;
@@ -86,8 +90,9 @@
     uint32_t pcap, hcap, nb;
     bool gaps, wide;
     bool nib;
+    bool snib;
     uint32_t off_heads, off_wb, off_ws;
-    uint32_t nib_wb, nib_ws;
+    uint32_t lds_wb, lds_ws;
     size_t lds;
     bool huge;
     uint32_t ntab;
@@ -97,9 +102,55 @@
 
 enum { PASS_MAIN = 0, PASS_BIG = 1, PASS_HUGE = 2 };
 
+using SearchFn = void (*)(SearchArgs);
+
+template <typename WT, int NT, typename IT, bool SN>
+static SearchFn search_kernel_nt(const LaunchPlan &P)
+{
+    if (P.nb <= 32) return P.gaps ? k_search<0, true, WT, NT, false, IT, SN> : k_search<0, false, WT, NT, false, IT, SN>;
+    if (P.nb <= 64) return P.gaps ? k_search<1, true, WT, NT, false, IT, SN> : k_search<1, false, WT, NT, false, IT, SN>;
+    return P.gaps ? k_search<2, true, WT, NT, false, IT, SN> : k_search<2, false, WT, NT, false, IT, SN>;
+}
+
+template <typename IT>
+static SearchFn search_kernel(const LaunchPlan &P)
+{
+    if (P.nib)
+        return P.nt == 64 ? search_kernel_nt<WNib, 64, IT, false>(P) : search_kernel_nt<WNib, 256, IT, false>(P);
+    if (P.snib)
+        return P.nt == 64 ? search_kernel_nt<uint8_t, 64, IT, true>(P) : search_kernel_nt<uint8_t, 256, IT, true>(P);
+    if (P.huge) {
+        if (P.wide) return P.gaps ? k_search<2, true, uint16_t, 64, true, IT> : k_search<2, false, uint16_t, 64, true, IT>;
+        return P.gaps ? k_search<2, true, uint8_t, 64, true, IT> : k_search<2, false, uint8_t, 64, true, IT>;
+    }
+    if (P.wide) return P.nt == 64 ? search_kernel_nt<uint16_t, 64, IT, false>(P) : search_kernel_nt<uint16_t, 256, IT, false>(P);
+    return P.nt == 64 ? search_kernel_nt<uint8_t, 64, IT, false>(P) : search_kernel_nt<uint8_t, 256, IT, false>(P);
+}
+
+static int kernel_waves_simd(SearchFn f)
+{
+    static std::mutex mu;
+    static std::map<SearchFn, int> known;
+    std::lock_guard<std::mutex> lock(mu);
+    const auto it = known.find(f);
+    if (it != known.end()) return it->second;
+    int w = HSA_WAVES_SIMD;
+    hipFuncAttributes at{};
+    if (hipFuncGetAttributes(&at, reinterpret_cast<const void *>(f)) == hipSuccess && at.numRegs > 0) {
+        w = 512 / ((at.numRegs + 7) / 8 * 8);
+        w = w > 8 ? 8 : w < 1 ? 1 : w;
+    } else {
+        (void)hipGetLastError();
+    }
+    known[f] = w;
+    return w;
+}
+
+template <typename IT = uint32_t>
 static int plan_launch(hsa_index *ix, int n_jobs, int max_len, int max_seed, const RegimePlan &R, int mode,
-                       LaunchPlan &P, uint32_t ent_bytes = 16)
-{
+                       LaunchPlan &P)
+{
+    constexpr uint32_t ent_bytes = 4u * sizeof(IT);
     const int nb = R.nb, max_entries = R.max_entries;
     const bool gaps = R.gaps, wide = R.wide, nib_ok = R.nib_ok;
     const bool big = mode == PASS_BIG;
@@ -110,19 +161,19 @@
     P.wide = wide;
     const uint32_t esz = wide ? 2u : 1u;
     P.nib = false;
+    P.snib = false;
     auto layout = [&](uint32_t nt) {
         const uint32_t epw = P.nib ? 8u : 4u / esz;
         P.nt = nt;
         P.off_heads = 2 * P.ntab + 128;
         P.off_wb = P.off_heads + (uint32_t)nb * nt * (P.huge ? 4u : 2u);
-        P.nib_wb = ((uint32_t)max_len + 7u) / 8u;
-        P.nib_ws = ((uint32_t)max_seed + 7u) / 8u;
-        const uint32_t wbw = P.nib ? P.nib_wb : (uint32_t)max_len / epw + 1u;
-        const uint32_t wsw = P.nib ? P.nib_ws : (uint32_t)max_seed / epw + 1u;
-        P.off_ws = P.off_wb + wbw * nt * 4u;
-        P.lds = ((size_t)P.off_ws + (size_t)wsw * nt * 4u + 15) / 16 * 16;
+        P.lds_wb = P.nib ? ((uint32_t)max_len + 7u) / 8u : P.snib ? ((uint32_t)max_len + 3u) / 4u : (uint32_t)max_len / epw + 1u;
+        P.lds_ws = P.nib || P.snib ? ((uint32_t)max_seed + 7u) / 8u : (uint32_t)max_seed / epw + 1u;
+        P.off_ws = P.off_wb + P.lds_wb * nt * 4u;
+        P.lds = ((size_t)P.off_ws + (size_t)P.lds_ws * nt * 4u + 15) / 16 * 16;
         int per_cu = (int)((160u * 1024u) / P.lds);
-        const int cap = 4 * HSA_WAVES_SIMD / (int)(nt / 64);
+        const int simd = P.snib ? kernel_waves_simd(search_kernel<IT>(P)) : HSA_WAVES_SIMD;
+        const int cap = 4 * simd / (int)(nt / 64);
         const int want = g_waves_per_cu / (int)(nt / 64);
         if (per_cu > cap) per_cu = cap;
         if (per_cu > want) per_cu = want > 0 ? want : 1;
@@ -131,7 +182,7 @@
     static const int force256 = getenv("HSA_WG256") != nullptr;
     auto best = [&]() {
         int per_cu = layout(P.huge ? 64 : 256);
-        if (per_cu < 4 && !force256 && !P.huge) {
+        if (!force256 && !P.huge) {
             const int p64 = layout(64);
             if (p64 > per_cu * 4) per_cu = p64;
             else per_cu = layout(256);
@@ -141,10 +192,21 @@
     int per_cu = best();
     const char *wf = getenv("HSA_WFMT");
     const bool force_nib = wf && !strcmp(wf, "nib"), no_nib = wf && !strcmp(wf, "byte");
-    if (nib_ok && !wide && !P.huge && !no_nib && (force_nib || (!gaps && per_cu * (int)(P.nt / 64) < 16))) {
+    const bool force_snib = wf && !strcmp(wf, "seednib");
+    if (R.snib_ok && !wide && !P.huge && !no_nib && max_seed > 0 && (force_snib || !gaps)) {
+        const int waves8 = per_cu * (int)(P.nt / 64);
+        const LaunchPlan keep = P;
+        P.snib = true;
+        const int per_sn = best();
+        if (!force_snib && per_sn * (int)(P.nt / 64) <= waves8) { P = keep; }
+        else per_cu = per_sn;
+    }
+    if (nib_ok && !wide && !P.huge && !no_nib && !force_snib &&
+        (force_nib || (!gaps && per_cu * (int)(P.nt / 64) < 16))) {
         const int waves8 = per_cu * (int)(P.nt / 64);
         const LaunchPlan keep = P;
         P.nib = true;
+        P.snib = false;
         const int per_nib = best();
         if (!force_nib && per_nib * (int)(P.nt / 64) <= waves8) { P = keep; }
         else per_cu = per_nib;
@@ -173,7 +235,7 @@
         (void)hipOccupancyMaxActiveBlocksPerMultiprocessor(&occ, k_search<1, true, uint8_t, 256>, 256, P.lds);
         fprintf(stderr, "[hsa] launch: %d CUs x %d workgroups of %u lanes (runtime occupancy query says %d), "
                 "LDS %zu B, %zu workgroups, %d buckets%s\n", ix->n_cu, per_cu, P.nt, occ, P.lds, blocks, nb,
-                P.nib ? ", 4-bit rows" : "");
+                P.nib ? ", 4-bit rows" : P.snib ? ", 4-bit seed row" : "");
     }
     static const int pool_env = getenv("HSA_POOL_ENTRIES") ? atoi(getenv("HSA_POOL_ENTRIES")) : 0;
     const int pool_main = g_pool_entries ? g_pool_entries : pool_env > 0 && pool_env <= 65535 ? pool_env : 0;
@@ -195,40 +257,10 @@
     return 0;
 }
 
-template <typename WT, int NT, typename IT>
-static void launch_search_nt(const LaunchPlan &P, const SearchArgs &A, hipStream_t st)
-{
-    const dim3 g((unsigned)P.blocks), b(NT);
-    if (P.nb <= 32) {
-        if (P.gaps) hipLaunchKernelGGL((k_search<0, true, WT, NT, false, IT>), g, b, P.lds, st, A);
-        else hipLaunchKernelGGL((k_search<0, false, WT, NT, false, IT>), g, b, P.lds, st, A);
-    } else if (P.nb <= 64) {
-        if (P.gaps) hipLaunchKernelGGL((k_search<1, true, WT, NT, false, IT>), g, b, P.lds, st, A);
-        else hipLaunchKernelGGL((k_search<1, false, WT, NT, false, IT>), g, b, P.lds, st, A);
-    } else {
-        if (P.gaps) hipLaunchKernelGGL((k_search<2, true, WT, NT, false, IT>), g, b, P.lds, st, A);
-        else hipLaunchKernelGGL((k_search<2, false, WT, NT, false, IT>), g, b, P.lds, st, A);
-    }
-}
-
-template <typename WT, typename IT>
+template <typename IT>
 static void launch_search(const LaunchPlan &P, const SearchArgs &A, hipStream_t st)
 {
-    if constexpr (!std::is_same<WT, WNib>::value) {
-        if (P.nib) {
-            if (P.nt == 64) launch_search_nt<WNib, 64, IT>(P, A, st);
-            else launch_search_nt<WNib, 256, IT>(P, A, st);
-            return;
-        }
-    }
-    if (P.huge) {
-        const dim3 g((unsigned)P.blocks), b(64);
-        if (P.gaps) hipLaunchKernelGGL((k_search<2, true, WT, 64, true, IT>), g, b, P.lds, st, A);
-        else hipLaunchKernelGGL((k_search<2, false, WT, 64, true, IT>), g, b, P.lds, st, A);
-        return;
-    }
-    if (P.nt == 64) launch_search_nt<WT, 64, IT>(P, A, st);
-    else launch_search_nt<WT, 256, IT>(P, A, st);
+    hipLaunchKernelGGL(search_kernel<IT>(P), dim3((unsigned)P.blocks), dim3(P.nt), P.lds, st, A);
 }
 
 static uint32_t trie_levels(const hsa_index *ix, bool wide)
@@ -271,7 +303,8 @@
     constexpr size_t WGB = sizeof(IT);
     const bool mg = io.mg.d_mg != nullptr;
     const uint32_t esz = P.wide ? 2u : 1u;
-    const uint32_t rb = (((uint32_t)io.max_len + 1u) * esz + 3u) & ~3u, rs = (((uint32_t)io.max_seed + 1u) * esz + 3u) & ~3u;
+    const uint32_t rb = (((uint32_t)io.max_len + 1u) * esz + 3u) & ~3u;
+    const uint32_t rs = P.snib ? ((uint32_t)io.max_seed / 8u + 1u) * 4u : (((uint32_t)io.max_seed + 1u) * esz + 3u) & ~3u;
     const uint32_t rg = (uint32_t)io.max_len + 1u;
     const size_t rows = ((size_t)io.n + 63) / 64 * 64 * 2;
     const size_t row_bytes = rb + rs + WGB * (size_t)rg + (mg ? 4 * (size_t)rg : 0);
@@ -294,7 +327,7 @@
     A.pool = S.pool; A.nxt = S.nxt; A.hbuf = S.hbuf;
     A.pcap = P.pcap; A.hcap = P.hcap;
     A.nb = P.nb; A.off_heads = P.off_heads; A.off_wb = P.off_wb; A.off_ws = P.off_ws;
-    A.nib_wb = P.nib_wb; A.nib_ws = P.nib_ws;
+    A.lds_wb = P.lds_wb; A.lds_ws = P.lds_ws;
     A.mm_buckets = ix->staged_mmb ? 1u : 0u;
     A.ntab = P.ntab;
     A.batch_k = (uint32_t)g_batch_k;
@@ -419,8 +452,7 @@
             else hipLaunchKernelGGL(k_widths_import<uint8_t>, dim3(nb ? nb : 1), dim3(BLOCK), 0, st, A);
             HSA_HIP(hipGetLastError());
             if (ix->ev_split) HSA_HIP(hipEventRecord(ix->ev_split, st));
-            if (P.wide) launch_search<uint16_t, uint32_t>(P, A, st);
-            else launch_search<uint8_t, uint32_t>(P, A, st);
+            launch_search<uint32_t>(P, A, st);
             HSA_HIP(hipGetLastError());
             hipLaunchKernelGGL(k_widths_export, dim3(nb ? nb : 1), dim3(BLOCK), 0, st, A);
             HSA_HIP(hipGetLastError());
@@ -473,6 +505,9 @@
         if (P.wide) {
             hipLaunchKernelGGL((k_widths_reads<uint16_t, IT>), dim3(rblocks), dim3(BLOCK), 0, st, A, 1u, d_list2, d_n2);
             hipLaunchKernelGGL((k_widths_reads<uint16_t, IT>), dim3(rblocks), dim3(BLOCK), 0, st, A, 3u, d_list2, d_n2);
+        } else if (P.snib) {
+            hipLaunchKernelGGL((k_widths_reads<uint8_t, IT, true>), dim3(rblocks), dim3(BLOCK), 0, st, A, 1u, d_list2, d_n2);
+            hipLaunchKernelGGL((k_widths_reads<uint8_t, IT, true>), dim3(rblocks), dim3(BLOCK), 0, st, A, 3u, d_list2, d_n2);
         } else {
             hipLaunchKernelGGL((k_widths_reads<uint8_t, IT>), dim3(rblocks), dim3(BLOCK), 0, st, A, 1u, d_list2, d_n2);
             hipLaunchKernelGGL((k_widths_reads<uint8_t, IT>), dim3(rblocks), dim3(BLOCK), 0, st, A, 3u, d_list2, d_n2);
@@ -481,6 +516,7 @@
         size_t wblocks = ((size_t)n * 2 + BLOCK - 1) / BLOCK;
         if (wblocks < 1) wblocks = 1;
         if (P.wide) hipLaunchKernelGGL((k_widths<uint16_t, IT>), dim3((unsigned)wblocks), dim3(BLOCK), 0, st, A);
+        else if (P.snib) hipLaunchKernelGGL((k_widths<uint8_t, IT, true>), dim3((unsigned)wblocks), dim3(BLOCK), 0, st, A);
         else hipLaunchKernelGGL((k_widths<uint8_t, IT>), dim3((unsigned)wblocks), dim3(BLOCK), 0, st, A);
     }
     HSA_HIP(hipGetLastError());
@@ -494,8 +530,7 @@
         A.perm = d_perm;
     }
     if (ix->ev_split && first) HSA_HIP(hipEventRecord(ix->ev_split, st));
-    if (P.wide) launch_search<uint16_t, IT>(P, A, st);
-    else launch_search<uint8_t, IT>(P, A, st);
+    launch_search<IT>(P, A, st);
     HSA_HIP(hipGetLastError());
     if (lazy) {
         SearchArgs F = A;
@@ -503,10 +538,10 @@
         F.fwd_list = nullptr; F.fwd_n = nullptr; F.wkey = nullptr; F.perm = nullptr; F.rmap = nullptr;
         const unsigned rblocks = (unsigned)(((size_t)n + BLOCK - 1) / BLOCK);
         if (P.wide) hipLaunchKernelGGL((k_widths_reads<uint16_t, IT>), dim3(rblocks), dim3(BLOCK), 0, st, F, 2u, d_list2, d_n2);
+        else if (P.snib) hipLaunchKernelGGL((k_widths_reads<uint8_t, IT, true>), dim3(rblocks), dim3(BLOCK), 0, st, F, 2u, d_list2, d_n2);
         else hipLaunchKernelGGL((k_widths_reads<uint8_t, IT>), dim3(rblocks), dim3(BLOCK), 0, st, F, 2u, d_list2, d_n2);
         HSA_HIP(hipGetLastError());
-        if (P.wide) launch_search<uint16_t, IT>(P, F, st);
-        else launch_search<uint8_t, IT>(P, F, st);
+        launch_search<IT>(P, F, st);
         HSA_HIP(hipGetLastError());
     }
     if (split) {
@@ -574,12 +609,11 @@
 static int run_capacity_passes(hsa_index *ix, const RegimePlan &C, const PassIO &io, PassLink main, bool zero_ctr,
                                hipEvent_t ev_split, hipStream_t st)
 {
-    constexpr uint32_t EB = 4u * sizeof(IT);
     LaunchPlan P, B, H;
     int rc;
-    if ((rc = plan_launch(ix, io.n, io.max_len, io.max_seed, C, PASS_MAIN, P, EB)) ||
-        (rc = plan_launch(ix, io.n, io.max_len, io.max_seed, C, PASS_BIG, B, EB)) ||
-        (rc = plan_launch(ix, io.n, io.max_len, io.max_seed, C, PASS_HUGE, H, EB)))
+    if ((rc = plan_launch<IT>(ix, io.n, io.max_len, io.max_seed, C, PASS_MAIN, P)) ||
+        (rc = plan_launch<IT>(ix, io.n, io.max_len, io.max_seed, C, PASS_BIG, B)) ||
+        (rc = plan_launch<IT>(ix, io.n, io.max_len, io.max_seed, C, PASS_HUGE, H)))
         return rc;
     if ((rc = hsa_grow(&ix->d_ovf, &ix->d_ovf_cap, (size_t)io.n * 4 + 64)) ||
         (rc = hsa_grow(&ix->d_ovf2, &ix->d_ovf2_cap, (size_t)io.n * 4 + 64)))
diff --git a/hsa_amd/csrc/hsa_splice_prefetch.h b/hsa_amd/csrc/hsa_splice_prefetch.h
--- a/hsa_amd/csrc/hsa_splice_prefetch.h
+++ b/hsa_amd/csrc/hsa_splice_prefetch.h
@@ -118,7 +118,7 @@
     S.jobs = (hsa_job_t *)d; S.mg = (hsa_mg_job_t *)(d + o_mg); S.codes = (uint8_t *)(d + o_codes);
     S.cw = (int32_t *)(d + o_cw); S.list = (int32_t *)(d + o_list); S.count = cnt; S.ctr = ctr;
     RegimePlan C = regime_plan(seed_regime, 1);
-    C.nib_ok = false;
+    C.nib_ok = false; C.snib_ok = false;
     if ((rc = stage_regimes(ix, seed_regime, 1, C.nb, st))) return rc;
     HSA_HIP(hipMemsetAsync(ctr, 0, CTR_SLOTS * sizeof(unsigned long long), st));
     hipLaunchKernelGGL(k_seed_prep, dim3((unsigned)((2 * n + BLOCK - 1) / BLOCK)), dim3(BLOCK), 0, st, S);
@@ -470,7 +470,7 @@
     const PfArgs &A = F.A;
     const PfLayout &L = F.L;
     RegimePlan C = regime_plan(anchors ? F.anchor_rg : F.seed_rg, 1);
-    C.nb = F.nb; C.wide = F.wide; C.nib_ok = false;
+    C.nb = F.nb; C.wide = F.wide; C.nib_ok = false; C.snib_ok = false;
     const PassIO io{.jobs = A.jobs, .list = A.list + (anchors ? 6 * (size_t)A.n : 0), .n = n_upper, .codes = A.scodes,
                     .n_aln = A.call_n, .flags = A.call_fl, .hit_off = F.at<uint64_t>(L.call_hit),
                     .hits = F.at<uint32_t>(anchors ? L.hits_a : L.hits_s), .hit_cap = anchors ? L.cap_a : L.cap_s,
```
